# microsoft/M3P

Measured on AMD Instinct MI355X. Metric: pre-train samples/sec (whole node), 12L/768d seq=128+36, higher is better.
Workload: dtype bf16; 1 GPU; cfg2: 12L/768d/12h, 36 regions + 128 tokens, V=250002, 19 MLM targets/seq + ITM BCE, dropout 0.10, adam_inverse_sqrt + clip 5; per_gpu_batch=256, global_batch=256, seq_len=164, parallelism=dp1, prewarm_steps=36

## Files before the change

include/m3p_hip.h:

```cpp
#ifndef M3P_HIP_H
#define M3P_HIP_H

#include <stddef.h>
#include <stdint.h>

#ifdef __cplusplus
extern "C" {
#endif

#define M3P_API __attribute__((visibility("default")))

#define M3P_OK 0
#define M3P_EINVAL (-1)
#define M3P_ENOTIMPL (-2)
#define M3P_ENOMEM (-3)

M3P_API const char* m3p_version(void);


enum {
  M3P_EPI_NONE = 0,
  M3P_EPI_BIAS = 1,
  M3P_EPI_BIAS_GELU = 2,
  M3P_EPI_BIAS_DROP_RES = 3,
  M3P_EPI_RES = 4,
  M3P_EPI_DGELU = 5,
  M3P_EPI_MUL = 6,
  M3P_EPI_MULQ = 7,
  M3P_EPI_BIAS_GELUQ = 8,
  M3P_EPI_BIAS_LSE = 9
};

typedef struct M3PEpilogue {
  const float* bias;
  const void* aux;
  void* out2;
  float* colsum;
  int32_t ld_aux;
  int32_t ld_out2;
  int32_t scale_cols;
  float scale;
  float alpha;
  uint32_t seed;
  uint32_t thresh24;
  float inv_keep;
  const float* descale_a;
  const float* descale_b;
  void* out8;
  const float* scale8;
  float* amax8;
  int32_t ld_out8;
  int32_t out8_bf8;
} M3PEpilogue;

M3P_API int m3p_gemm_nt_bf16(const void* A, int lda, const void* W, int ldw, void* C, int ldc,
                             int M, int N, int K, int epilogue, const M3PEpilogue* ep, void* stream);

M3P_API int m3p_gemm_nt_fp8(const void* A8, int lda, int a_is_bf8, const void* W8, int ldw, void* C, int ldc,
                            int M, int N, int K, int epilogue, const M3PEpilogue* ep, void* stream);

M3P_API int m3p_quant_fp8(const void* src, int ld_src, void* dst, int ld_dst, int rows, int cols, const float* scale,
                          float* amax, int bf8, void* stream);

M3P_API int m3p_quant_fp8_batch(const long long* desc, int n_desc, int blocks_per_matrix, void* stream);

M3P_API int m3p_gemm_nt_streamk_f32(const void* A, int lda, const void* W, int ldw, float* C, int ldc,
                                    int M, int N, int K, float alpha, void* stream);
M3P_API int m3p_gemm_nn_streamk_f32(const void* A, int lda, const void* W, int ldw, int k_valid, float* C,
                                    int ldc, int M, int N, int K, float alpha, void* stream);
M3P_API int m3p_gemm_nn_w4_f32(const void* A, int lda, const void* W, int ldw, float* C, int ldc, int M, int N, int K, float alpha,
                               void* workspace, size_t workspace_bytes, void* stream);

M3P_API size_t m3p_gemm_wgrad_workspace_bytes(void);
M3P_API int m3p_gemm_wgrad_bf16(const void* dY, int lddy, const void* X, int ldx, float* dW, int lddw,
                                int M, int N, int K, float alpha, void* workspace, size_t workspace_bytes,
                                void* stream);
M3P_API int m3p_gemm_wgrad_store_bf16(const void* dY, int lddy, const void* X, int ldx, float* dW, int lddw, int M, int N, int K,
                                      float alpha, void* workspace, size_t workspace_bytes, void* stream);
M3P_API int m3p_gemm_wgrad_pair_bf16(const void* dYa, int lddya, const void* Xa, int ldxa, float* dWa, int lddwa, int Na, int Ka,
                                     const void* dYb, int lddyb, const void* Xb, int ldxb, float* dWb, int lddwb, int Nb, int Kb,
                                     int M, float alpha, void* workspace, size_t workspace_bytes, void* stream);


M3P_API int m3p_layernorm_fwd(const void* x, const float* gamma, const float* beta, const uint8_t* rowmask,
                              void* y, float* mean, float* rstd, int rows, int d, float eps, void* stream);

M3P_API int m3p_layernorm_bwd(const void* dy_a, const void* dy_b, const void* x, const float* gamma,
                              const float* mean, const float* rstd, const uint8_t* rowmask,
                              void* dx, void* dx_drop, float* dgamma, float* dbeta, float* dbias_drop,
                              int rows, int d, uint32_t seed, uint32_t thresh24, float inv_keep, void* stream);


M3P_API int m3p_attn_fwd(const void* qkv, const int32_t* keylen, void* ctx, float* lse, uint64_t* keepmask,
                         int B, int S, int H, int dh, uint32_t seed, uint32_t thresh24, float inv_keep,
                         void* stream);

M3P_API int m3p_attn_bwd(const void* qkv, const int32_t* keylen, const void* ctx, const void* dctx,
                         const float* lse, const uint64_t* keepmask, void* dqkv, float* dbias_qkv, int B, int S,
                         int H, int dh, float qscale, uint32_t seed, uint32_t thresh24, float inv_keep,
                         void* stream);

M3P_API int m3p_attn_query_fwd(const void* q, int ld_q, const void* kv, long long kv_bstride, int ld_kv,
                               const int32_t* klen, void* ctx, int B, int Tq, int H, int dh, int Lk, int causal,
                               int pos0, void* stream);

M3P_API int m3p_attn_rows_fwd(const void* q, int ld_q, const void* kv, long long kv_bstride, int ld_kv, const int32_t* klen,
                              void* ctx, float* lse, int B, int Tq, int H, int dh, int Lk, int causal, int pos0,
                              uint32_t seed, uint32_t thresh24, float inv_keep, void* stream);
M3P_API int m3p_attn_rows_bwd(const void* q, int ld_q, const void* kv, long long kv_bstride, int ld_kv, const int32_t* klen,
                              const void* dctx, const float* lse, void* dq, int ld_dq, float* dkv, int B, int Tq, int H,
                              int dh, int Lk, int causal, int pos0, float qscale, uint32_t seed, uint32_t thresh24,
                              float inv_keep, void* stream);


M3P_API int m3p_cast_f32_bf16(const float* src, void* dst, long long n, void* stream);

M3P_API int m3p_embed_assemble_fwd(const int64_t* tok, const void* emb_bf16, const float* pos,
                                   const void* img_proj, const float* loc, const float* w_loc,
                                   const float* b_loc, const float* g_img, const float* be_img,
                                   const float* g_emb, const float* be_emb, const int32_t* totlen,
                                   void* h, void* z, float* mean_emb, float* rstd_emb, void* e,
                                   float* mean_img, float* rstd_img, int B, int T, int R, int d,
                                   uint32_t seed_img, uint32_t seed_emb, uint32_t thresh24, float inv_keep,
                                   const void* img_rows, void* stream);

M3P_API int m3p_embed_image_rows_fwd(const void* img_proj, const float* loc, const float* w_loc, const float* b_loc,
                                     const float* g_img, const float* be_img, void* e, float* mean_img,
                                     float* rstd_img, void* img_rows, int B, int R, int d, uint32_t seed_img,
                                     uint32_t thresh24, float inv_keep, void* stream);

M3P_API int m3p_embed_assemble_bwd(const void* dh, const void* z, const float* mean_emb, const float* rstd_emb,
                                   const float* g_emb, const void* e, const float* mean_img,
                                   const float* rstd_img, const float* g_img, const int64_t* tok,
                                   const int32_t* totlen, const float* loc, void* dz_scratch, void* de,
                                   float* d_g_emb, float* d_be_emb, float* d_pos, float* d_emb,
                                   void* d_tok_rows, float* d_g_img, float* d_be_img, float* d_b_img, float* d_b_loc,
                                   float* d_w_loc, int B, int T, int R, int d, int pad_index,
                                   uint32_t seed_img, uint32_t seed_emb, uint32_t thresh24, float inv_keep,
                                   int phase, void* stream);


M3P_API int m3p_gather_rows(const void* src, const int32_t* idx, void* dst, int n, int d, void* stream);
M3P_API int m3p_scatter_add_rows(const void* src, const int32_t* idx, void* dst, int n, int d, void* stream);
M3P_API int m3p_scatter_add_token_rows(const void* rows, int ld_rows, const int64_t* ids, float* dst, int n, int d,
                                       int pad_index, void* stream);

M3P_API int m3p_itm_score_fwd(const void* pre, const float* w2, const float* b2, float* pooled, float* scores, int B,
                              int d, void* stream);
M3P_API int m3p_itm_score_bwd(const float* dscores, const float* pooled, const float* w2, void* dpre16, void* dpreT16,
                              int ldt, float* db1, float* dw2, float* db2, int B, int d, void* stream);

M3P_API int m3p_ce_fwd_bwd(void* logits, int ld, int n_rows, int V, const int64_t* target, float* row_loss,
                           float* loss_sum, float loss_scale, float grad_scale, void* stream);

M3P_API int m3p_ce_lse_from_blocks(const void* stats, int n_blocks, int n_rows, const void* logits, int ld, const int64_t* target,
                                   float* row_loss, float* row_lse, void* scratch, void* stream);
M3P_API int m3p_ce_bwd_colsum(void* logits, int ld, int n_rows, int V, const int64_t* target, const float* row_lse,
                              float grad_scale, float* colsum, void* workspace, size_t workspace_bytes, void* stream);
M3P_API size_t m3p_ce_colsum_workspace_bytes(int ld, int n_rows);
M3P_API int m3p_ce_fwd_bwd_colsum(void* logits, int ld, int n_rows, int V, const int64_t* target, float* row_loss,
                                  float* row_lse, float grad_scale, float* colsum, void* workspace,
                                  size_t workspace_bytes, void* stream);

M3P_API int m3p_colsum_bf16(const void* x, int ld, int n, int ncols, float* out, const float* scale_ptr,
                            void* stream);


M3P_API int m3p_sumsq_f32(const float* g, long long n, double* out, void* stream);

M3P_API int m3p_sumsq_ranges_f32(const float* base, const long long* starts, const long long* counts, int n_ranges, double* out,
                                 void* stream);

M3P_API int m3p_adam_step(float* p, float* g, float* m, float* v, void* w16, long long n, float lr, float beta1,
                          float beta2, float eps, float weight_decay, float step_size, const double* gnorm_sq,
                          float max_norm, float grad_scale, int zero_grad, void* stream);
M3P_API int m3p_adam_step_ranges(float* p, float* g, float* m, float* v, void* w16, const long long* starts,
                                 const long long* counts, const float* step_sizes, const int* zero_grad, int n_ranges,
                                 float lr, float beta1, float beta2, float eps, float weight_decay, const double* gnorm_sq,
                                 float max_norm, float grad_scale, void* stream);

M3P_API int m3p_gelu_fwd(const void* u, void* h, void* dh, long long n, void* stream);
M3P_API int m3p_gelu_fwd_gq(const void* u, void* h, void* gq, int M, int N, void* stream);
M3P_API int m3p_gelu_fwd_q8(const void* u, void* h, void* h8, long long n, const float* scale, float* amax, void* stream);

M3P_API int m3p_gelu_bwd(const void* dy, const void* u, void* du, long long n, void* stream);

M3P_API int m3p_mse_fwd_bwd(const void* pred, int ld_pred, const float* tgt, int ld_tgt, void* dpred, float* row_sq,
                            int rows, int cols, float grad_scale, void* stream);


M3P_API int m3p_dropout_rows(const void* x, int ldx, const void* res, int ldres, void* y, int ldy, int rows, int cols,
                             uint32_t rng_ld, uint32_t rng_col0, uint32_t seed, uint32_t thresh24, float inv_keep,
                             void* stream);

M3P_API int m3p_glu_fwd(const void* ab, int ld_ab, void* y, int rows, int d, void* stream);
// ... 51 lines not shown
```

m3p_amd/csrc/gemm.hip:

```cpp
#include <mutex>
#include <type_traits>
#include "common.hpp"
#include "../../include/m3p_hip.h"
#include <hip/amd_detail/amd_hip_unsafe_atomics.h>

static int g_variant = 1;
extern "C" void m3p_debug_set_variant(int v) { g_variant = (v == 2 || v == 6) ? v : 1; }

namespace {

constexpr int BK = 64;
constexpr int ROWB = BK * 2;

template <int EPI>
__device__ __forceinline__ void epilogue_store(const M3PEpilogue& ep, bf16* __restrict__ C, int ldc,
                                               int M, int N, int m, int n, f32x4 acc, f32x4& csum) {
  if (m >= M || n >= N) return;
  const bool full = (n + 3 < N);
  float v[4] = {acc[0], acc[1], acc[2], acc[3]};
  const float alpha = (ep.alpha == 0.f) ? 1.f : ep.alpha;
  if (EPI == M3P_EPI_NONE || EPI == M3P_EPI_BIAS || EPI == M3P_EPI_RES) {
#pragma unroll
    for (int r = 0; r < 4; ++r) v[r] *= alpha;
  }
  if (EPI == M3P_EPI_BIAS || EPI == M3P_EPI_BIAS_GELU || EPI == M3P_EPI_BIAS_DROP_RES) {
    if (ep.bias) {
#pragma unroll
      for (int r = 0; r < 4; ++r)
        if (n + r < N) v[r] += ep.bias[n + r];
    }
  }
  if (EPI == M3P_EPI_BIAS) {
#pragma unroll
    for (int r = 0; r < 4; ++r)
      if (n + r < ep.scale_cols) v[r] *= ep.scale;
  }
  if (EPI == M3P_EPI_BIAS_GELU) {
    bf16* U = reinterpret_cast<bf16*>(ep.out2) + (size_t)m * ep.ld_out2 + n;
    bf16 ur[4];
#pragma unroll
    for (int r = 0; r < 4; ++r) { ur[r] = (bf16)v[r]; v[r] = gelu_erf_f((float)ur[r]); }
    if (full) *reinterpret_cast<bf16x4*>(U) = bf16x4{ur[0], ur[1], ur[2], ur[3]};
    else
      for (int r = 0; r < 4; ++r) if (n + r < N) U[r] = ur[r];
  }
  if (EPI == M3P_EPI_BIAS_DROP_RES) {
    if (ep.thresh24) {
      const uint32_t base = (uint32_t)m * (uint32_t)N + (uint32_t)n;
      bool kp[4];
      m3p_keep_run<4>(base, ep.seed, ep.thresh24, kp);
#pragma unroll
      for (int r = 0; r < 4; ++r) v[r] = kp[r] ? v[r] * ep.inv_keep : 0.f;
    }
  }
  if (EPI == M3P_EPI_BIAS_DROP_RES || EPI == M3P_EPI_RES || EPI == M3P_EPI_DGELU || EPI == M3P_EPI_MUL) {
    const bf16* X = reinterpret_cast<const bf16*>(ep.aux) + (size_t)m * ep.ld_aux + n;
    float a[4] = {0.f, 0.f, 0.f, 0.f};
    if (full) { bf16x4 t = *reinterpret_cast<const bf16x4*>(X); a[0] = (float)t[0]; a[1] = (float)t[1]; a[2] = (float)t[2]; a[3] = (float)t[3]; }
    else
      for (int r = 0; r < 4; ++r) if (n + r < N) a[r] = (float)X[r];
    if (EPI == M3P_EPI_DGELU) {
#pragma unroll
      for (int r = 0; r < 4; ++r) v[r] *= gelu_erf_grad_f(a[r]);
    } else if (EPI == M3P_EPI_MUL) {
#pragma unroll
      for (int r = 0; r < 4; ++r) v[r] *= a[r];
    } else {
#pragma unroll
      for (int r = 0; r < 4; ++r) v[r] += a[r];
    }
  }
  bf16 o[4];
#pragma unroll
  for (int r = 0; r < 4; ++r) o[r] = (bf16)v[r];
  bf16* Cp = C + (size_t)m * ldc + n;
  if (full) *reinterpret_cast<bf16x4*>(Cp) = bf16x4{o[0], o[1], o[2], o[3]};
  else
    for (int r = 0; r < 4; ++r) if (n + r < N) Cp[r] = o[r];
  if (EPI == M3P_EPI_DGELU || EPI == M3P_EPI_MUL) {
#pragma unroll
    for (int r = 0; r < 4; ++r) csum[r] += (n + r < N) ? (float)o[r] : 0.f;
  }
}

template <int BM, int BN, int EPI>
__global__ __launch_bounds__(64 * (BM / 64) * (BN / 64))
void gemm_nt_kernel(const bf16* __restrict__ A, int lda, const bf16* __restrict__ W, int ldw,
                    bf16* __restrict__ C, int ldc, int M, int N, int K, M3PEpilogue ep,
                    int tiles_m, int tiles_n) {
  constexpr int WAVES_M = BM / 64, WAVES_N = BN / 64, NWAVES = WAVES_M * WAVES_N;
  constexpr int A_BYTES = BM * ROWB, B_BYTES = BN * ROWB, STAGE = A_BYTES + B_BYTES;
  extern __shared__ __attribute__((aligned(16))) char smem[];

  const int tid = threadIdx.x, lane = tid & 63;
  const int wid = __builtin_amdgcn_readfirstlane(tid >> 6);
  const int id = xcd_remap(blockIdx.x, tiles_m * tiles_n);
  const int tm = id / tiles_n, tn = id - tm * tiles_n;
  const int m0 = tm * BM, n0 = tn * BN;

  const int sr = lane >> 3, sc = (lane & 7) ^ sr;
  const bf16* a_src[BM / 8 / NWAVES];
// ... 150 lines not shown
template <class P>
__device__ __forceinline__ void st16(P* p, const u32x4& v) {
  *reinterpret_cast<u32x4*>(p) = v;
}
template <bool NT>
__device__ __forceinline__ void st16p(void* p, const u32x4& v) {
  if (NT) __builtin_nontemporal_store(v, reinterpret_cast<u32x4*>(p));
  else *reinterpret_cast<u32x4*>(p) = v;
}
template <int EPI>
__device__ __forceinline__ void load_aux_rows_issue(const M3PEpilogue& ep, int mrow0, int nw, int lane, u32x4 (&t)[4]) {
  constexpr bool kAux = (EPI == M3P_EPI_BIAS_DROP_RES || EPI == M3P_EPI_RES || EPI == M3P_EPI_DGELU || EPI == M3P_EPI_MUL);
  if (!kAux) return;
  const int srow = lane >> 3, sch = lane & 7;
  const bf16* X = reinterpret_cast<const bf16*>(ep.aux) + (size_t)(mrow0 + srow) * ep.ld_aux + nw + sch * 8;
#pragma unroll
  for (int it = 0; it < 4; ++it) {
    t[it] = *reinterpret_cast<const u32x4*>(X + (size_t)(it * 8) * ep.ld_aux);
  }
}
template <int EPI, bool SW = false, bool ALDS = false>
__device__ __forceinline__ void load_aux_rows_finish(int lane, char* r1, const u32x4 (&t)[4], bf16x4 (&auxv)[2][4]) {
  constexpr bool kAux = (EPI == M3P_EPI_BIAS_DROP_RES || EPI == M3P_EPI_RES || EPI == M3P_EPI_DGELU || EPI == M3P_EPI_MUL);
  if (!kAux) return;
  const int srow = lane >> 3, sch = lane & 7;
  const int fr = lane & 15, fg = lane >> 4;
  if (ALDS) {
    const uint32_t la = lds_addr(r1);
#pragma unroll
    for (int it = 0; it < 4; ++it) lds_w128(la + ep_off<SW>(it * 8 + srow, sch * 16), flip_halves(t[it], SW && (it & 1)));
#pragma unroll
    for (int ii = 0; ii < 2; ++ii)
#pragma unroll
      for (int j = 0; j < 4; ++j) lds_r64(la + ep_off8<SW>(ii * 16 + fr, (j * 16 + fg * 4) * 2), auxv[ii][j]);
    asm volatile("s_waitcnt lgkmcnt(0)" : "+v"(auxv[0][0]), "+v"(auxv[0][1]), "+v"(auxv[0][2]), "+v"(auxv[0][3]),
                                         "+v"(auxv[1][0]), "+v"(auxv[1][1]), "+v"(auxv[1][2]), "+v"(auxv[1][3]));
    return;
  }
#pragma unroll
  for (int it = 0; it < 4; ++it) *reinterpret_cast<u32x4*>(r1 + ep_off<SW>(it * 8 + srow, sch * 16)) = flip_halves(t[it], SW && (it & 1));
#pragma unroll
  for (int ii = 0; ii < 2; ++ii)
#pragma unroll
    for (int j = 0; j < 4; ++j)
      auxv[ii][j] = *reinterpret_cast<const bf16x4*>(r1 + ep_off8<SW>(ii * 16 + fr, (j * 16 + fg * 4) * 2));
}
template <int EPI, bool SW = false>
__device__ __forceinline__ void load_aux_rows(const M3PEpilogue& ep, int mrow0, int nw, int lane, char* r1, bf16x4 (&auxv)[2][4]) {
  u32x4 t[4];
  load_aux_rows_issue<EPI>(ep, mrow0, nw, lane, t);
  load_aux_rows_finish<EPI, SW>(lane, r1, t, auxv);
}

template <int EPI, bool SW = false, bool ALDS = false>
__device__ __forceinline__ void epilogue_half_write(const M3PEpilogue& ep, int N, int mrow0, int nw, char* r1, const f32x4 (&rows)[2][4],
                                                    const f32x4 (&biasv)[4], const bf16x4 (&auxv)[2][4], int lane, f32x4 (&csum)[4],
                                                    bf16x4 (&ukeep)[2][4], const float* gtab = nullptr) {
  const int fr = lane & 15, fg = lane >> 4;
  constexpr bool kAux = (EPI == M3P_EPI_BIAS_DROP_RES || EPI == M3P_EPI_RES || EPI == M3P_EPI_DGELU || EPI == M3P_EPI_MUL);
  const float alpha = (ep.alpha == 0.f) ? 1.f : ep.alpha;
#pragma unroll
  for (int j = 0; j < 4; ++j) {
    const int n = nw + j * 16 + fg * 4;
    f32x4 bias4 = biasv[j];
    f32x4 mulc = {alpha, alpha, alpha, alpha};
    if (EPI == M3P_EPI_BIAS) {
#pragma unroll
      for (int r = 0; r < 4; ++r)
        if (n + r < ep.scale_cols) { mulc[r] *= ep.scale; bias4[r] *= ep.scale; }
    }
#pragma unroll
    for (int ii = 0; ii < 2; ++ii) {
      const int rl = ii * 16 + fr;
      const int mrow = mrow0 + rl;
      const int lo = ep_off8<SW>(rl, (j * 16 + fg * 4) * 2);
      f32x4 v = rows[ii][j];
      if (EPI == M3P_EPI_NONE || EPI == M3P_EPI_BIAS || EPI == M3P_EPI_RES) v = v * mulc + bias4;
      else if (EPI != M3P_EPI_DGELU && EPI != M3P_EPI_MUL) v += bias4;
      if (EPI == M3P_EPI_BIAS_GELU) {
        ukeep[ii][j] = bf16x4{(bf16)v[0], (bf16)v[1], (bf16)v[2], (bf16)v[3]};
#pragma unroll
        for (int r = 0; r < 4; ++r) v[r] = gelu_erf_f((float)ukeep[ii][j][r]);
      }
      if (EPI == M3P_EPI_BIAS_DROP_RES && ep.thresh24) {
        const uint32_t base = (uint32_t)mrow * (uint32_t)N + (uint32_t)n;
        bool kp[4];
        m3p_keep_even<4>(base, ep.seed, ep.thresh24, kp);
#pragma unroll
        for (int r = 0; r < 4; ++r) v[r] = kp[r] ? v[r] * ep.inv_keep : 0.f;
      }
      if (kAux) {
        const bf16x4 t = auxv[ii][j];
        const f32x4 a = f32x4{(float)t[0], (float)t[1], (float)t[2], (float)t[3]};
        if (EPI == M3P_EPI_DGELU) {
          if (gtab) {
#pragma unroll
            for (int r = 0; r < 4; ++r) v[r] *= gelu_grad_lookup(gtab, t[r]);
          } else {
#pragma unroll
            for (int r = 0; r < 4; ++r) v[r] *= gelu_erf_grad_f(a[r]);
          }
        } else if (EPI == M3P_EPI_MUL) {
          v *= a;
        } else {
          v += a;
        }
      }
      const bf16x4 ob = bf16x4{(bf16)v[0], (bf16)v[1], (bf16)v[2], (bf16)v[3]};
      if (ALDS) lds_w64(lds_addr(r1) + lo, ob);
      else *reinterpret_cast<bf16x4*>(r1 + lo) = ob;
      if (EPI == M3P_EPI_DGELU || EPI == M3P_EPI_MUL) csum[j] += f32x4{(float)ob[0], (float)ob[1], (float)ob[2], (float)ob[3]};
    }
  }
}
template <bool SW>
__device__ __forceinline__ void epilogue_rows_read(const char* r1, int lane, u32x4 (&R)[4]) {
  const int srow = lane >> 3, sch = lane & 7;
  const uint32_t la = lds_addr(r1);
#pragma unroll
  for (int it = 0; it < 4; ++it) lds_r128(la + ep_off<SW>(it * 8 + srow, sch * 16), R[it]);
}
template <bool SW>
__device__ __forceinline__ void lgkm_wait_rows(u32x4 (&R)[4], bool younger8) {
  if (younger8) asm volatile("s_waitcnt lgkmcnt(8)" : "+v"(R[0]), "+v"(R[1]), "+v"(R[2]), "+v"(R[3]));
  else asm volatile("s_waitcnt lgkmcnt(0)" : "+v"(R[0]), "+v"(R[1]), "+v"(R[2]), "+v"(R[3]));
#pragma unroll
  for (int it = 0; it < 4; ++it) R[it] = flip_halves(R[it], SW && (it & 1));
}
__device__ __forceinline__ void epilogue_rows_store(bf16* __restrict__ C, int ldc, int mrow0, int nw, int lane, const u32x4 (&R)[4]) {
  const int srow = lane >> 3, sch = lane & 7;
  bf16* Cp = C + (size_t)mrow0 * ldc + nw + sch * 8;
#pragma unroll
  for (int it = 0; it < 4; ++it) st16(Cp + (size_t)(it * 8 + srow) * ldc, R[it]);
}
template <int EPI, bool SW = false>
__device__ __forceinline__ void epilogue_half(const M3PEpilogue& ep, bf16* __restrict__ C, int ldc, int N,
                                              int mrow0, int nw, char* r1, const f32x4 (&rows)[2][4],
                                              const f32x4 (&biasv)[4], const bf16x4 (&auxv)[2][4], int lane, f32x4 (&csum)[4],
// ... 1364 lines not shown
  } else {
    asm volatile("s_waitcnt vmcnt(0)" ::: "memory");
  }
  __builtin_amdgcn_s_barrier();
  asm volatile("" ::: "memory");
  bf16x8 af0[4], wf0[4], af1[4], wf1[4];
  s16x4 wh0[4][2], wh1[4][2];
  read_set(0, 0, af0, wf0, wh0);
  M3P_LGKM0();
  WgCursor cc = locate(g0l);
  int cur = 0;
  for (int step = 0; step < total; ++step) {
    const int nxt = (cur == 2) ? 0 : cur + 1;
    const int nx2 = (nxt == 2) ? 0 : nxt + 1;
    const bool more2 = (step + 2 < total);
    if (more2) stage_next(nx2);
    read_set(1, cur * STAGE, af1, wf1, wh1);
    __builtin_amdgcn_sched_barrier(0);
    mfma_batch(af0, wf0, wh0);
    M3P_LGKM0();
    if (more2) asm volatile("s_waitcnt vmcnt(6)" ::: "memory");
    else asm volatile("s_waitcnt vmcnt(0)" ::: "memory");
    __builtin_amdgcn_s_barrier();
    asm volatile("" ::: "memory");
    __builtin_amdgcn_sched_barrier(0);
    read_set(0, nxt * STAGE, af0, wf0, wh0);
    __builtin_amdgcn_sched_barrier(0);
    mfma_batch(af1, wf1, wh1);
    M3P_LGKM0();
    if ((cc.mt + 1 == cc.len) || (step + 1 == total)) {
      const int tm = cc.t / tiles_n, tn = cc.t - tm * tiles_n;
#pragma unroll
      for (int i = 0; i < 4; ++i) {
        const int m = tm * BM + wm * 64 + i * 16 + fr;
#pragma unroll
        for (int j = 0; j < 4; ++j) {
          const int n = tn * BN + wn * 64 + j * 16 + fg * 4;
#pragma unroll
          for (int r = 0; r < 4; ++r) {
            if (m < M && n + r < N) unsafeAtomicAdd(Cf + (size_t)m * ldc + n + r, alpha * acc[i][j][r]);
            acc[i][j][r] = 0.f;
          }
        }
      }
    }
    advance(cc);
    cur = nxt;
  }
#undef M3P_DSR
#undef M3P_TRH
#undef M3P_LGKM0
}

template <int EPI>
__global__ __launch_bounds__(256)
void gemm_nt_w4_kernel(const bf16* __restrict__ A, int lda, const bf16* __restrict__ W, int ldw,
                       bf16* __restrict__ C, int ldc, int M, int N, int K, M3PEpilogue ep,
                       int tiles_m, int tiles_n, int m_fast) {
  constexpr int BM = 256, BN = 256, KT = 64;
  constexpr int A_BYTES = BM * KT * 2, STAGE = (BM + BN) * KT * 2;
  extern __shared__ __attribute__((aligned(16))) char smem[];

  const int tid = threadIdx.x, lane = tid & 63;
  const int wid = __builtin_amdgcn_readfirstlane(tid >> 6);
  const int ntiles = tiles_m * tiles_n;
  const int n_strips = (tiles_n >= 12) ? (tiles_n + 3) / 4 : 1;
  const int strip_w = (tiles_n + n_strips - 1) / n_strips;
  auto split_tile = [&](int t, int& tm, int& tn) {
    if (m_fast) { tn = t / tiles_m; tm = t - tn * tiles_m; return; }
    const int strip = t / (tiles_m * strip_w);
    const int rem = t - strip * tiles_m * strip_w;
    const int bn = min(strip_w, tiles_n - strip * strip_w);
    tm = rem / bn;
    tn = strip * strip_w + (rem - tm * bn);
  };
  const int nwg = gridDim.x;
  const int per_xcd = nwg >> 3;
  const int slot = (blockIdx.x & 7) * per_xcd + (blockIdx.x >> 3);
  auto tile_of = [&](int q) { return q * nwg + slot; };
  const int my_tiles = (ntiles > slot) ? (ntiles - slot + nwg - 1) / nwg : 0;
  if (my_tiles == 0) return;
  const int nk = K / KT;
  const int total = my_tiles * nk;

  const int l_row = lane >> 3;
  const int l_col = ((lane & 7) ^ l_row) * 8;
  const uint32_t a_lane = (uint32_t)(l_row * lda + l_col) * 2u, w_lane = (uint32_t)(l_row * ldw + l_col) * 2u;
  __amdgpu_buffer_rsrc_t a_rsrc, w_rsrc;
  int l_q = 0, l_kt = 0;
  auto set_load_tile = [&](int q) {
    int tm, tn;
    split_tile(tile_of(q), tm, tn);
    const bf16* a_tile = A + (size_t)(tm * BM + wid * 64) * lda;
    const bf16* w_tile = W + (size_t)(tn * BN + wid * 64) * ldw;
    a_rsrc = __builtin_amdgcn_make_buffer_rsrc(const_cast<bf16*>(uniform_ptr(a_tile)), 0, 0xffffffff, 0x00020000);
    w_rsrc = __builtin_amdgcn_make_buffer_rsrc(const_cast<bf16*>(uniform_ptr(w_tile)), 0, 0xffffffff, 0x00020000);
  };
#define W4_LDB(IMM) __builtin_amdgcn_raw_ptr_buffer_load_lds(piece < 8 ? a_rsrc : w_rsrc, LDS_PTR(sl), 16, piece < 8 ? a_lane : w_lane, soff, IMM, 0)
  auto issue_load = [&](int s, int piece) {
    const int pc = piece & 7;
    char* sl = smem + s * STAGE + (piece < 8 ? 0 : A_BYTES) + wid * 8192 + (pc >> 2) * 4096;
    const uint32_t k_off = (uint32_t)l_kt * (KT * 2);
    const uint32_t soff = __builtin_amdgcn_readfirstlane(k_off + (uint32_t)pc * (uint32_t)((piece < 8 ? lda : ldw) * 16) - (uint32_t)(pc & 3) * 1024u);
    switch (pc & 3) {
      case 0: W4_LDB(0); break;
      case 1: W4_LDB(1024); break;
      case 2: W4_LDB(2048); break;
      default: W4_LDB(3072); break;
    }
  };
  auto load_done = [&]() {
// ... 204 lines not shown
        load_bias4<EPI>(ep, btn * BN + wn * 128 + 64, lane, bias_hi);
      }
      ktile(std::true_type{}, stage_c);
    } else {
      ktile(std::false_type{}, stage_c);
    }
    if (++c_kt == nk) {
      c_kt = 0;
      asm volatile("s_nop 15\n\ts_nop 15" ::: "memory");
      int tm, tn;
      split_tile(tile_of(c_q), tm, tn);
      ++c_q;
      const int m0 = tm * BM, n0 = tn * BN;
      const int mw = m0 + wm * 128, nw = n0 + wn * 128;
      const bool fast = io_aligned && (m0 + BM <= M) && (n0 + BN <= N);
      f32x4 csum[4];
#pragma unroll
      for (int j = 0; j < 4; ++j) csum[j] = f32x4{0.f, 0.f, 0.f, 0.f};
#define W4_RD(II, JJ, I, J)                                                         \
  asm volatile("v_accvgpr_read_b32 %0, a[((" #I ")*8+(" #J "))*4+0]\n\t"            \
               "v_accvgpr_read_b32 %1, a[((" #I ")*8+(" #J "))*4+1]\n\t"            \
               "v_accvgpr_read_b32 %2, a[((" #I ")*8+(" #J "))*4+2]\n\t"            \
               "v_accvgpr_read_b32 %3, a[((" #I ")*8+(" #J "))*4+3]"                \
               : "=v"(t0), "=v"(t1), "=v"(t2), "=v"(t3));                           \
  rows[II][JJ] = f32x4{t0, t1, t2, t3}
#define W4_SLICE(RG, CH)                                                                      \
  W4_RD(0, 0, 2 * RG, 4 * CH); W4_RD(0, 1, 2 * RG, 4 * CH + 1); W4_RD(0, 2, 2 * RG, 4 * CH + 2); W4_RD(0, 3, 2 * RG, 4 * CH + 3); \
  W4_RD(1, 0, 2 * RG + 1, 4 * CH); W4_RD(1, 1, 2 * RG + 1, 4 * CH + 1); W4_RD(1, 2, 2 * RG + 1, 4 * CH + 2); W4_RD(1, 3, 2 * RG + 1, 4 * CH + 3)
      constexpr bool kPipe = (EPI == M3P_EPI_NONE || EPI == M3P_EPI_BIAS || EPI == M3P_EPI_RES || EPI == M3P_EPI_BIAS_DROP_RES);
      if (kPipe && fast) {
        char* rb = smem + 2 * STAGE + wid * EP_HALF;
        u32x4 tq[4];
        load_aux_rows_issue<EPI>(ep, mw, nw, lane, tq);
#pragma nounroll
        for (int p = 0; p < 8; ++p) {
          const int ch = p >> 2, rg = p & 3;
          f32x4 rows[2][4];
          float t0, t1, t2, t3;
          switch (p) {
            case 0: W4_SLICE(0, 0); break;
            case 1: W4_SLICE(1, 0); break;
            case 2: W4_SLICE(2, 0); break;
            case 3: W4_SLICE(3, 0); break;
            case 4: W4_SLICE(0, 1); break;
            case 5: W4_SLICE(1, 1); break;
            case 6: W4_SLICE(2, 1); break;
            default: W4_SLICE(3, 1); break;
          }
          char* rc = rb;
          bf16x4 aux_cur[2][4];
          load_aux_rows_finish<EPI, true, true>(lane, rc, tq, aux_cur);
          if (p + 1 < 8) load_aux_rows_issue<EPI>(ep, mw + 32 * ((p + 1) & 3), nw + 64 * ((p + 1) >> 2), lane, tq);
          bf16x4 ukeep[2][4];
          epilogue_half_write<EPI, true, true>(ep, N, mw + 32 * rg, nw + 64 * ch, rc, rows, ch ? bias_hi : bias_lo, aux_cur, lane, csum, ukeep);
          u32x4 R[4];
          epilogue_rows_read<true>(rc, lane, R);
          lgkm_wait_rows<true>(R, false);
          epilogue_rows_store(C, ldc, mw + 32 * rg, nw + 64 * ch, lane, R);
        }
      } else
#pragma nounroll
      for (int p = 0; p < 8; ++p) {
        const int ch = p >> 2, rg = p & 3;
        bf16x4 aux_cur[2][4];
        if (fast) {
          if (EPI == M3P_EPI_DGELU || EPI == M3P_EPI_MUL) load_aux<EPI>(ep, mw + 32 * rg, nw + 64 * ch, lane, aux_cur);
          else load_aux_rows<EPI>(ep, mw + 32 * rg, nw + 64 * ch, lane, r1, aux_cur);
        }
        f32x4 rows[2][4];
        float t0, t1, t2, t3;
        switch (p) {
          case 0: W4_SLICE(0, 0); break;
          case 1: W4_SLICE(1, 0); break;
          case 2: W4_SLICE(2, 0); break;
          case 3: W4_SLICE(3, 0); break;
          case 4: W4_SLICE(0, 1); break;
          case 5: W4_SLICE(1, 1); break;
          case 6: W4_SLICE(2, 1); break;
          default: W4_SLICE(3, 1); break;
        }
        const int mrow0 = mw + 32 * rg, ncol0 = nw + 64 * ch;
        if (fast) {
          epilogue_half<EPI>(ep, C, ldc, N, mrow0, ncol0, r1, rows, ch ? bias_hi : bias_lo, aux_cur, lane, csum);
        } else {
#pragma unroll
          for (int ii = 0; ii < 2; ++ii)
#pragma unroll
            for (int jj = 0; jj < 4; ++jj)
              epilogue_store<EPI>(ep, C, ldc, M, N, mrow0 + ii * 16 + fr, ncol0 + jj * 16 + fg * 4, rows[ii][jj], csum[jj]);
        }
        if ((EPI == M3P_EPI_DGELU || EPI == M3P_EPI_MUL) && rg == 3) {
          if (ep.colsum) {
#pragma unroll
            for (int j = 0; j < 4; ++j)
#pragma unroll
              for (int r = 0; r < 4; ++r) {
                float sfl = csum[j][r];
                sfl += __shfl_xor(sfl, 1, 64); sfl += __shfl_xor(sfl, 2, 64);
                sfl += __shfl_xor(sfl, 4, 64); sfl += __shfl_xor(sfl, 8, 64);
                const int n = ncol0 + j * 16 + fg * 4 + r;
                if (fr == 0 && n < N) unsafeAtomicAdd(ep.colsum + n, sfl);
              }
          }
#pragma unroll
          for (int j = 0; j < 4; ++j) csum[j] = f32x4{0.f, 0.f, 0.f, 0.f};
        }
      }
// ... 141 lines not shown
int launch_nt(const bf16* A, int lda, const bf16* W, int ldw, bf16* C, int ldc, int M, int N, int K,
              const M3PEpilogue& ep, hipStream_t st) {
  int want_queue = 0;
  const int plan = nt_plan(EPI, M, N, K, &want_queue);
  if (plan == M3P_KERN_NT_SKINNY) {
    if constexpr (EPI != M3P_EPI_DGELU && EPI != M3P_EPI_MUL) {
      if (M <= 16) return launch_nt_skinny<EPI, 1>(A, lda, W, ldw, C, ldc, M, N, K, ep, st);
      if (M <= 32) return launch_nt_skinny<EPI, 2>(A, lda, W, ldw, C, ldc, M, N, K, ep, st);
      if (M <= 64) return launch_nt_skinny<EPI, 4>(A, lda, W, ldw, C, ldc, M, N, K, ep, st);
      return launch_nt_skinny<EPI, 8>(A, lda, W, ldw, C, ldc, M, N, K, ep, st);
    }
  }
  if (plan == M3P_KERN_NT_W8) {
    const int tiles_m = M / 256, tiles_n = N / 256;
    const size_t lds = 2 * 512 * ROWB + (EPI == M3P_EPI_DGELU ? GELU_TAB_N * sizeof(float) : 0) +
                       ((EPI == M3P_EPI_DGELU || EPI == M3P_EPI_MUL) ? 8 * 2048 : 8 * 4096);
    auto kern = gemm_nt_w8_kernel<EPI>;
    static bool attr_set8 = false;
    if (!attr_set8) {
      hipError_t e = hipFuncSetAttribute((const void*)kern, hipFuncAttributeMaxDynamicSharedMemorySize, (int)lds);
      if (e != hipSuccess) return (int)e;
      attr_set8 = true;
    }
    int grid = num_cus();
    const int ntiles = tiles_m * tiles_n;
    if (ntiles < grid) grid = (ntiles + 7) / 8 * 8;
    constexpr bool kQueueOk = !(EPI == M3P_EPI_DGELU || EPI == M3P_EPI_MUL);
    int* ctr = nullptr;
    if (kQueueOk && want_queue) {
      hipError_t e;
      ctr = tq_acquire(st, &e);
      if (e != hipSuccess) return (int)e;
    }
    if constexpr (kQueueOk) if (ctr) {
      auto kern_d = gemm_nt_w8_kernel<EPI, true>;
      static bool attr_set8d = false;
      if (!attr_set8d) {
        hipError_t e = hipFuncSetAttribute((const void*)kern_d, hipFuncAttributeMaxDynamicSharedMemorySize, (int)lds);
        if (e != hipSuccess) return (int)e;
        attr_set8d = true;
      }
      hipLaunchKernelGGL(kern_d, dim3(grid), dim3(512), lds, st, A, lda, W, ldw, C, ldc, M, N, K, ep, tiles_m, tiles_n, ctr);
      M3P_CHECK_LAUNCH();
      return M3P_OK;
    }
    hipLaunchKernelGGL(kern, dim3(grid), dim3(512), lds, st, A, lda, W, ldw, C, ldc, M, N, K, ep, tiles_m, tiles_n, ctr);
    M3P_CHECK_LAUNCH();
    return M3P_OK;
  }
  if (plan == M3P_KERN_NT_W4) {
    constexpr int BM = 256, BN = 256;
    const int tiles_m = (M + BM - 1) / BM, tiles_n = (N + BN - 1) / BN;
    const size_t lds = 2 * (BM + BN) * 128 + 4 * EP_HALF;
    auto kern = gemm_nt_w4_kernel<EPI>;
    static bool attr_set = false;
    if (!attr_set) {
      hipError_t e = hipFuncSetAttribute((const void*)kern, hipFuncAttributeMaxDynamicSharedMemorySize, (int)lds);
      if (e != hipSuccess) return (int)e;
      attr_set = true;
    }
    int grid = num_cus();
    const int ntiles = tiles_m * tiles_n;
    if (ntiles < grid) grid = (ntiles + 7) / 8 * 8;
    const long long wbytes = 2LL * N * K, abytes = 2LL * M * K;
    const int m_fast = (wbytes > (64LL << 20) && abytes < wbytes) ? 1 : 0;
    hipLaunchKernelGGL(kern, dim3(grid), dim3(256), lds, st, A, lda, W, ldw, C, ldc, M, N, K, ep, tiles_m, tiles_n, m_fast);
    M3P_CHECK_LAUNCH();
    return M3P_OK;
  }
  if (plan == M3P_KERN_NT_RING) {
    constexpr int BM = 256, BN = 128;
    const int tiles_m = (M + BM - 1) / BM, tiles_n = (N + BN - 1) / BN;
    const size_t lds = 3 * (BM + BN) * ROWB + (EPI == M3P_EPI_DGELU ? GELU_TAB_N * sizeof(float) : 0);
    auto kern = gemm_nt_ring_kernel<EPI>;
    static bool attr_set = false;
    if (!attr_set) {
      hipError_t e = hipFuncSetAttribute((const void*)kern, hipFuncAttributeMaxDynamicSharedMemorySize, (int)lds);
      if (e != hipSuccess) return (int)e;
      attr_set = true;
    }
    int grid = num_cus();
    const int ntiles = tiles_m * tiles_n;
    if (ntiles < grid) grid = (ntiles + 7) / 8 * 8;
    hipLaunchKernelGGL(kern, dim3(grid), dim3(512), lds, st, A, lda, W, ldw, C, ldc, M, N, K, ep, tiles_m, tiles_n);
    M3P_CHECK_LAUNCH();
    return M3P_OK;
  }
  constexpr int BM = 128, BN = 128;
  const int tiles_m = (M + BM - 1) / BM, tiles_n = (N + BN - 1) / BN;
  const size_t lds = 2 * (BM + BN) * ROWB;
  auto kern = gemm_nt_kernel<BM, BN, EPI>;
  static bool attr_set = false;
  if (!attr_set) {
    hipError_t e = hipFuncSetAttribute((const void*)kern, hipFuncAttributeMaxDynamicSharedMemorySize, (int)lds);
    if (e != hipSuccess) return (int)e;
    attr_set = true;
  }
  hipLaunchKernelGGL(kern, dim3(tiles_m * tiles_n), dim3(256), lds, st, A, lda, W, ldw, C, ldc, M, N, K, ep,
                     tiles_m, tiles_n);
  M3P_CHECK_LAUNCH();
  return M3P_OK;
}

template <int EPI>
static int launch_nt_gq(const bf16* A, int lda, const bf16* W, int ldw, bf16* C, int ldc, int M, int N, int K,
                        const M3PEpilogue& ep, hipStream_t st) {
  if (M < 1024 || (M % 256) || (N % 256) || N < 512 || (K % 64) || (lda % 8) || (ldw % 8) || (ldc % 8) || ((uintptr_t)C & 15))
    return M3P_EINVAL;
// ... 1081 lines not shown
```

m3p_amd/csrc/heads.hip:

```cpp
#include "common.hpp"
#include <hip/amd_detail/amd_hip_unsafe_atomics.h>

namespace {

__global__ __launch_bounds__(256) void gather_rows_kernel(const bf16* __restrict__ src, const int32_t* __restrict__ idx,
                                                          bf16* __restrict__ dst, int n, int d) {
  const int nchunk = d >> 2;
  const size_t total = (size_t)n * nchunk;
  for (size_t i = (size_t)blockIdx.x * blockDim.x + threadIdx.x; i < total; i += (size_t)gridDim.x * blockDim.x) {
    const int r = (int)(i / nchunk), c = (int)(i - (size_t)r * nchunk);
    *reinterpret_cast<bf16x4*>(dst + (size_t)r * d + 4 * c) =
        *reinterpret_cast<const bf16x4*>(src + (size_t)idx[r] * d + 4 * c);
  }
}
__global__ __launch_bounds__(256) void scatter_add_rows_kernel(const bf16* __restrict__ src, const int32_t* __restrict__ idx,
                                                               bf16* __restrict__ dst, int n, int d) {
  const int nchunk = d >> 2;
  const size_t total = (size_t)n * nchunk;
  for (size_t i = (size_t)blockIdx.x * blockDim.x + threadIdx.x; i < total; i += (size_t)gridDim.x * blockDim.x) {
    const int r = (int)(i / nchunk), c = (int)(i - (size_t)r * nchunk);
    bf16* p = dst + (size_t)idx[r] * d + 4 * c;
    Vec4<bf16>::store(p, Vec4<bf16>::load(p) + Vec4<bf16>::load(src + (size_t)r * d + 4 * c));
  }
}

__global__ __launch_bounds__(256) void scatter_add_token_rows_kernel(const bf16* __restrict__ rows, int ld_rows, const int64_t* __restrict__ ids,
                                                                     float* __restrict__ dst, int n, int d, int pad_index) {
  const int lane = threadIdx.x & 63;
  const int wave = (int)((blockIdx.x * blockDim.x + threadIdx.x) >> 6), nwave = (int)((gridDim.x * blockDim.x) >> 6);
  for (int r = wave; r < n; r += nwave) {
    const int64_t id = ids[r];
    if (id == pad_index) continue;
    const bf16* src = rows + (size_t)r * ld_rows;
    float* out = dst + (size_t)id * d;
    for (int e = lane; e < d; e += 64) {
      const float v = (float)src[e];
      if (v != 0.f) unsafeAtomicAdd(out + e, v);
    }
  }
}

__global__ __launch_bounds__(1024) void ce_fwd_bwd_kernel(bf16* __restrict__ logits, int ld, int V,
                                                          const int64_t* __restrict__ target, float* __restrict__ row_loss,
                                                          float* __restrict__ loss_sum, float loss_scale, float gscale) {
  __shared__ float s_m[16], s_s[16];
  constexpr float kLog2e = 1.4426950408889634f;
  const int row = blockIdx.x, tid = threadIdx.x, lane = tid & 63, wib = tid >> 6;
  bf16* lr = logits + (size_t)row * ld;
  const int nchunk = ld >> 3;
  float m = -INFINITY, s = 0.f;
  for (int c = tid; c < nchunk; c += 1024) {
    const bf16x8 v = *reinterpret_cast<const bf16x8*>(lr + 8 * c);
    float x[8];
    float gm = -INFINITY;
#pragma unroll
    for (int j = 0; j < 8; ++j) {
      x[j] = (8 * c + j < V) ? (float)v[j] : -INFINITY;
      gm = fmaxf(gm, x[j]);
    }
    if (gm > m) {
      s *= __builtin_amdgcn_exp2f((m - gm) * kLog2e);
      m = gm;
    }
    const float mb = m * kLog2e;
#pragma unroll
// ... 219 lines not shown

int m3p_ce_lse_from_blocks(const void* stats, int n_blocks, int n_rows, const void* logits, int ld, const int64_t* target,
                           float* row_loss, float* row_lse, void* scratch, void* stream) {
  if (n_blocks <= 0 || n_rows <= 0 || (n_rows % 64) != 0 || !stats || !logits || !target || !row_loss || !row_lse || !scratch ||
      ((uintptr_t)stats & 7) || ((uintptr_t)scratch & 7))
    return M3P_EINVAL;
  hipStream_t st = (hipStream_t)stream;
  hipLaunchKernelGGL(ce_lse_partial_kernel, dim3(n_rows / 64, CE_LSE_SPLIT), dim3(256), 0, st, (const float2*)stats, n_blocks, n_rows,
                     (float2*)scratch);
  hipLaunchKernelGGL(ce_lse_final_kernel, dim3((n_rows + 255) / 256), dim3(256), 0, st, (const float2*)scratch, n_rows,
                     (const bf16*)logits, ld, target, row_loss, row_lse);
  M3P_CHECK_LAUNCH();
  return M3P_OK;
}

int m3p_ce_bwd_colsum(void* logits, int ld, int n_rows, int V, const int64_t* target, const float* row_lse,
                      float grad_scale, float* colsum, void* workspace, size_t workspace_bytes, void* stream) {
  if (n_rows <= 0 || V <= 0 || ld < V || (ld % 8) != 0 || ((uintptr_t)logits & 15) || ((uintptr_t)colsum & 15) ||
      ((uintptr_t)workspace & 15) || !row_lse)
    return M3P_EINVAL;
  if (workspace_bytes < m3p_ce_colsum_workspace_bytes(ld, n_rows)) return M3P_EINVAL;
  hipStream_t st = (hipStream_t)stream;
  const int groups = (n_rows + CE_RB - 1) / CE_RB;
  hipLaunchKernelGGL(ce_grad_tile_kernel, dim3((ld + CE_CB - 1) / CE_CB, groups), dim3(256), 0, st, (bf16*)logits, ld, n_rows, V,
                     target, (const float*)row_lse, grad_scale, (float*)workspace);
  if (hipMemsetAsync(colsum, 0, (size_t)ld * sizeof(float), st) != hipSuccess) return M3P_EINVAL;
  hipLaunchKernelGGL(ce_colsum_reduce_kernel, dim3((ld / 4 + 255) / 256, groups >= 16 ? 8 : 1), dim3(256), 0, st,
                     (const float*)workspace, ld, groups, colsum);
  M3P_CHECK_LAUNCH();
  return M3P_OK;
}

int m3p_colsum_bf16(const void* x, int ld, int n, int ncols, float* out, const float* scale_ptr, void* stream) {
  if (n <= 0 || ncols <= 0 || (ld % 4) != 0 || ld < ((ncols + 3) / 4) * 4) return M3P_EINVAL;
  const int c4 = (ncols + 3) / 4;
  int ysplit = 1;
  while (ysplit < 64 && ((c4 + 255) / 256) * ysplit < 1024 && n / (ysplit * 2) >= 16) ysplit *= 2;
  hipLaunchKernelGGL(colsum_kernel, dim3((c4 + 255) / 256, ysplit), dim3(256), 0, (hipStream_t)stream, (const bf16*)x, ld,
                     n, ncols, out, scale_ptr);
  M3P_CHECK_LAUNCH();
  return M3P_OK;
}

int m3p_gather_rows(const void* src, const int32_t* idx, void* dst, int n, int d, void* stream) {
  if (n <= 0) return M3P_OK;
  if ((d % 4) != 0) return M3P_EINVAL;
  const size_t total = (size_t)n * (d / 4);
  const int blocks = (int)((total + 255) / 256 < 2048 ? (total + 255) / 256 : 2048);
  hipLaunchKernelGGL(gather_rows_kernel, dim3(blocks), dim3(256), 0, (hipStream_t)stream, (const bf16*)src, idx, (bf16*)dst, n, d);
  M3P_CHECK_LAUNCH();
  return M3P_OK;
}

int m3p_scatter_add_rows(const void* src, const int32_t* idx, void* dst, int n, int d, void* stream) {
  if (n <= 0) return M3P_OK;
  if ((d % 4) != 0) return M3P_EINVAL;
  const size_t total = (size_t)n * (d / 4);
  const int blocks = (int)((total + 255) / 256 < 2048 ? (total + 255) / 256 : 2048);
  hipLaunchKernelGGL(scatter_add_rows_kernel, dim3(blocks), dim3(256), 0, (hipStream_t)stream, (const bf16*)src, idx, (bf16*)dst, n, d);
  M3P_CHECK_LAUNCH();
  return M3P_OK;
}

int m3p_scatter_add_token_rows(const void* rows, int ld_rows, const int64_t* ids, float* dst, int n, int d, int pad_index, void* stream) {
  if (n <= 0) return M3P_OK;
  if (d <= 0 || ld_rows < d) return M3P_EINVAL;
  const int blocks = (n + 3) / 4 < 4096 ? (n + 3) / 4 : 4096;
  hipLaunchKernelGGL(scatter_add_token_rows_kernel, dim3(blocks), dim3(256), 0, (hipStream_t)stream, (const bf16*)rows, ld_rows, ids,
                     dst, n, d, pad_index);
  M3P_CHECK_LAUNCH();
  return M3P_OK;
}

int m3p_ce_fwd_bwd(void* logits, int ld, int n_rows, int V, const int64_t* target, float* row_loss, float* loss_sum,
                   float loss_scale, float grad_scale, void* stream) {
  if (n_rows <= 0 || V <= 0 || ld < V || (ld % 8) != 0 || ((uintptr_t)logits & 15)) return M3P_EINVAL;
  hipLaunchKernelGGL(ce_fwd_bwd_kernel, dim3(n_rows), dim3(1024), 0, (hipStream_t)stream, (bf16*)logits, ld, V, target,
                     row_loss, loss_sum, loss_scale, grad_scale);
  M3P_CHECK_LAUNCH();
  return M3P_OK;
}

}
```

m3p_amd/csrc/layernorm.hip:

```cpp
#include "common.hpp"
#include "../../include/m3p_hip.h"
#include <hip/amd_detail/amd_hip_unsafe_atomics.h>

namespace {

constexpr int LN_BWD_BLOCKS = 512;

template <int NI>
__global__ __launch_bounds__(256)
void ln_fwd_kernel(const bf16* __restrict__ x, const float* __restrict__ gamma, const float* __restrict__ beta,
                   const uint8_t* __restrict__ rowmask, bf16* __restrict__ y, float* __restrict__ mean,
                   float* __restrict__ rstd, int rows, int d, float eps) {
  const int lane = threadIdx.x & 63;
  const int wave = (blockIdx.x * blockDim.x + threadIdx.x) >> 6;
  const int nwaves = (gridDim.x * blockDim.x) >> 6;
  const int nchunk = d >> 2;
  const float inv_d = 1.0f / (float)d;

  f32x4 g[NI], b[NI];
#pragma unroll
  for (int i = 0; i < NI; ++i) {
    const int c = lane + 64 * i;
    if (c < nchunk) { g[i] = Vec4<float>::load(gamma + 4 * c); b[i] = Vec4<float>::load(beta + 4 * c); }
  }
  for (int r = wave; r < rows; r += nwaves) {
    const bf16* xr = x + (size_t)r * d;
    f32x4 v[NI];
    float s = 0.f;
#pragma unroll
    for (int i = 0; i < NI; ++i) {
      const int c = lane + 64 * i;
      v[i] = f32x4{0.f, 0.f, 0.f, 0.f};
      if (c < nchunk) v[i] = Vec4<bf16>::load(xr + 4 * c);
      s += (v[i][0] + v[i][1]) + (v[i][2] + v[i][3]);
    }
    const float mu = wave_sum(s) * inv_d;
    float q = 0.f;
#pragma unroll
    for (int i = 0; i < NI; ++i) {
      const int c = lane + 64 * i;
      if (c < nchunk) {
        const f32x4 t = v[i] - mu;
        q += (t[0] * t[0] + t[1] * t[1]) + (t[2] * t[2] + t[3] * t[3]);
      }
    }
    const float rs = 1.0f / sqrtf(wave_sum(q) * inv_d + eps);
    const float mk = rowmask ? (rowmask[r] ? 1.f : 0.f) : 1.f;
    bf16* yr = y + (size_t)r * d;
#pragma unroll
    for (int i = 0; i < NI; ++i) {
      const int c = lane + 64 * i;
      if (c < nchunk) {
        f32x4 o = ((v[i] - mu) * rs * g[i] + b[i]) * mk;
        Vec4<bf16>::store(yr + 4 * c, o);
      }
    }
    if (lane == 0) { mean[r] = mu; rstd[r] = rs; }
  }
}

template <int NI>
__global__ __launch_bounds__(256)
void ln_bwd_kernel(const bf16* __restrict__ dy_a, const bf16* __restrict__ dy_b, const bf16* __restrict__ x,
                   const float* __restrict__ gamma, const float* __restrict__ mean, const float* __restrict__ rstd,
                   const uint8_t* __restrict__ rowmask, bf16* __restrict__ dx, bf16* __restrict__ dx_drop,
                   float* __restrict__ dgamma, float* __restrict__ dbeta, float* __restrict__ dbias_drop,
                   int rows, int d, uint32_t seed, uint32_t thresh24, float inv_keep) {
  __shared__ float red[4][NI * 256];
  const int lane = threadIdx.x & 63, wib = threadIdx.x >> 6;
  const int wave = (blockIdx.x * blockDim.x + threadIdx.x) >> 6;
  const int nwaves = (gridDim.x * blockDim.x) >> 6;
  const int nchunk = d >> 2;
  const float inv_d = 1.0f / (float)d;

  f32x4 g[NI], acc_g[NI], acc_b[NI], acc_d[NI];
#pragma unroll
  for (int i = 0; i < NI; ++i) {
    const int c = lane + 64 * i;
    g[i] = f32x4{0.f, 0.f, 0.f, 0.f};
    if (c < nchunk) g[i] = Vec4<float>::load(gamma + 4 * c);
    acc_g[i] = acc_b[i] = acc_d[i] = f32x4{0.f, 0.f, 0.f, 0.f};
  }
  for (int r = wave; r < rows; r += nwaves) {
    const size_t ro = (size_t)r * d;
    const float mu = mean[r], rs = rstd[r];
    const float mk = rowmask ? (rowmask[r] ? 1.f : 0.f) : 1.f;
    f32x4 dyv[NI], xh[NI];
    float s1 = 0.f, s2 = 0.f;
#pragma unroll
    for (int i = 0; i < NI; ++i) {
      const int c = lane + 64 * i;
      dyv[i] = xh[i] = f32x4{0.f, 0.f, 0.f, 0.f};
      if (c < nchunk) {
        dyv[i] = Vec4<bf16>::load(dy_a + ro + 4 * c);
        if (dy_b) dyv[i] += Vec4<bf16>::load(dy_b + ro + 4 * c);
        dyv[i] *= mk;
        xh[i] = (Vec4<bf16>::load(x + ro + 4 * c) - mu) * rs;
        const f32x4 gd = dyv[i] * g[i];
        s1 += (gd[0] + gd[1]) + (gd[2] + gd[3]);
        const f32x4 gx = gd * xh[i];
        s2 += (gx[0] + gx[1]) + (gx[2] + gx[3]);
        acc_g[i] += dyv[i] * xh[i];
        acc_b[i] += dyv[i];
      }
    }
    const float c1 = wave_sum(s1) * inv_d, c2 = wave_sum(s2) * inv_d;
#pragma unroll
    for (int i = 0; i < NI; ++i) {
      const int c = lane + 64 * i;
      if (c < nchunk) {
        const f32x4 o = (dyv[i] * g[i] - c1 - xh[i] * c2) * rs;
        Vec4<bf16>::store(dx + ro + 4 * c, o);
        if (dx_drop || dbias_drop) {
          bf16x4 ob = bf16x4{(bf16)o[0], (bf16)o[1], (bf16)o[2], (bf16)o[3]};
          f32x4 od;
          const uint32_t base = (uint32_t)r * (uint32_t)d + 4u * (uint32_t)c;
          bool kp[4] = {true, true, true, true};
          if (thresh24) m3p_keep_even<4>(base, seed, thresh24, kp);
#pragma unroll
          for (int e = 0; e < 4; ++e) od[e] = kp[e] ? (float)ob[e] * (thresh24 ? inv_keep : 1.f) : 0.f;
          bf16x4 odb = bf16x4{(bf16)od[0], (bf16)od[1], (bf16)od[2], (bf16)od[3]};
          if (dx_drop) *reinterpret_cast<bf16x4*>(dx_drop + ro + 4 * c) = odb;
          acc_d[i] += f32x4{(float)odb[0], (float)odb[1], (float)odb[2], (float)odb[3]};
        }
      }
    }
  }
  float* const outs[3] = {dgamma, dbeta, dbias_drop};
#pragma unroll
  for (int q = 0; q < 3; ++q) {
    if (outs[q] == nullptr) continue;
#pragma unroll
    for (int i = 0; i < NI; ++i) {
      const int col = 4 * (lane + 64 * i);
      const f32x4 a = (q == 0) ? acc_g[i] : (q == 1) ? acc_b[i] : acc_d[i];
#pragma unroll
      for (int e = 0; e < 4; ++e) red[wib][col + e] = a[e];
    }
    __syncthreads();
    for (int c = threadIdx.x; c < d; c += blockDim.x)
      unsafeAtomicAdd(outs[q] + c, (red[0][c] + red[1][c]) + (red[2][c] + red[3][c]));
    __syncthreads();
  }
}

template <int NC>
__global__ __launch_bounds__(256)
void ln_bwd_hw_kernel(const bf16* __restrict__ dy_a, const bf16* __restrict__ dy_b, const bf16* __restrict__ x,
                      const float* __restrict__ gamma, const float* __restrict__ mean, const float* __restrict__ rstd,
                      const uint8_t* __restrict__ rowmask, bf16* __restrict__ dx, bf16* __restrict__ dx_drop,
                      float* __restrict__ dgamma, float* __restrict__ dbeta, float* __restrict__ dbias_drop,
                      int rows, uint32_t seed, uint32_t thresh24, float inv_keep) {
  constexpr int D = 256 * NC;
  __shared__ float red[8][D];
  const int sub = threadIdx.x & 31, hw = threadIdx.x >> 5;
  const int ghw = blockIdx.x * 8 + hw, nhw = gridDim.x * 8;
  const float inv_d = 1.0f / (float)D;
  float g[NC][8], acc_g[NC][8], acc_b[NC][8], acc_d[NC][8];
#pragma unroll
  for (int i = 0; i < NC; ++i) {
    const int c = (sub + 32 * i) * 8;
    const f32x4 g0 = Vec4<float>::load(gamma + c), g1 = Vec4<float>::load(gamma + c + 4);
#pragma unroll
    for (int e = 0; e < 4; ++e) { g[i][e] = g0[e]; g[i][4 + e] = g1[e]; }
#pragma unroll
    for (int e = 0; e < 8; ++e) acc_g[i][e] = acc_b[i][e] = acc_d[i][e] = 0.f;
  }
  auto hsum = [](float v) {
#pragma unroll
    for (int o = 16; o > 0; o >>= 1) v += __shfl_xor(v, o, 64);
    return v;
  };
  for (int r = ghw; r < rows; r += nhw) {
    const size_t ro = (size_t)r * D;
    const float mu = mean[r], rs = rstd[r];
    const float mk = rowmask ? (rowmask[r] ? 1.f : 0.f) : 1.f;
    float dyv[NC][8], xh[NC][8];
    float s1 = 0.f, s2 = 0.f;
#pragma unroll
    for (int i = 0; i < NC; ++i) {
      const int c = (sub + 32 * i) * 8;
      bf16x8 a = *reinterpret_cast<const bf16x8*>(dy_a + ro + c);
      const bf16x8 xv = *reinterpret_cast<const bf16x8*>(x + ro + c);
      bf16x8 b2;
      if (dy_b) b2 = *reinterpret_cast<const bf16x8*>(dy_b + ro + c);
#pragma unroll
      for (int e = 0; e < 8; ++e) {
        float dv = (float)a[e];
        if (dy_b) dv += (float)b2[e];
        dv *= mk;
        const float xe = ((float)xv[e] - mu) * rs;
        dyv[i][e] = dv; xh[i][e] = xe;
        const float gd = dv * g[i][e];
        s1 += gd; s2 += gd * xe;
        acc_g[i][e] += dv * xe;
        acc_b[i][e] += dv;
      }
    }
    const float c1 = hsum(s1) * inv_d, c2 = hsum(s2) * inv_d;
#pragma unroll
    for (int i = 0; i < NC; ++i) {
      const int c = (sub + 32 * i) * 8;
      bf16x8 ob, odb;
#pragma unroll
      for (int e = 0; e < 8; ++e) ob[e] = (bf16)((dyv[i][e] * g[i][e] - c1 - xh[i][e] * c2) * rs);
      *reinterpret_cast<bf16x8*>(dx + ro + c) = ob;
      if (dx_drop || dbias_drop) {
        const uint32_t base = (uint32_t)r * (uint32_t)D + (uint32_t)c;
        bool kp[8] = {true, true, true, true, true, true, true, true};
        if (thresh24) m3p_keep_even<8>(base, seed, thresh24, kp);
#pragma unroll
        for (int e = 0; e < 8; ++e) {
          odb[e] = (bf16)(kp[e] ? (float)ob[e] * (thresh24 ? inv_keep : 1.f) : 0.f);
          acc_d[i][e] += (float)odb[e];
        }
        if (dx_drop) *reinterpret_cast<bf16x8*>(dx_drop + ro + c) = odb;
      }
    }
  }
  float* const outs[3] = {dgamma, dbeta, dbias_drop};
#pragma unroll
  for (int q = 0; q < 3; ++q) {
    if (outs[q] == nullptr) continue;
#pragma unroll
    for (int i = 0; i < NC; ++i) {
      const int c = (sub + 32 * i) * 8;
#pragma unroll
      for (int e = 0; e < 8; ++e) red[hw][c + e] = (q == 0) ? acc_g[i][e] : (q == 1) ? acc_b[i][e] : acc_d[i][e];
    }
    __syncthreads();
    for (int c = threadIdx.x; c < D; c += 256) {
      float t = 0.f;
#pragma unroll
      for (int w = 0; w < 8; ++w) t += red[w][c];
      unsafeAtomicAdd(outs[q] + c, t);
    }
    __syncthreads();
  }
}

inline int ln_ni(int d) { return (d + 255) / 256; }

}

extern "C" {

int m3p_layernorm_fwd(const void* x, const float* gamma, const float* beta, const uint8_t* rowmask, void* y,
                      float* mean, float* rstd, int rows, int d, float eps, void* stream) {
  if (rows <= 0 || d <= 0 || (d % 4) != 0 || d > 2048) return M3P_EINVAL;
  if (((uintptr_t)x & 7) || ((uintptr_t)y & 7) || ((uintptr_t)gamma & 15) || ((uintptr_t)beta & 15)) return M3P_EINVAL;
  const int blocks = min((rows + 3) / 4, 4096);
  hipStream_t st = (hipStream_t)stream;
#define M3P_LN_FWD(NI)                                                                                  \
  hipLaunchKernelGGL(ln_fwd_kernel<NI>, dim3(blocks), dim3(256), 0, st, (const bf16*)x, gamma, beta,    \
                     rowmask, (bf16*)y, mean, rstd, rows, d, eps)
  switch (ln_ni(d)) {
    case 1: M3P_LN_FWD(1); break;
    case 2: M3P_LN_FWD(2); break;
    case 3: M3P_LN_FWD(3); break;
    case 4: M3P_LN_FWD(4); break;
    default: M3P_LN_FWD(8); break;
  }
#undef M3P_LN_FWD
  M3P_CHECK_LAUNCH();
  return M3P_OK;
}

int m3p_layernorm_bwd(const void* dy_a, const void* dy_b, const void* x, const float* gamma, const float* mean,
                      const float* rstd, const uint8_t* rowmask, void* dx, void* dx_drop, float* dgamma,
                      float* dbeta, float* dbias_drop, int rows, int d, uint32_t seed, uint32_t thresh24,
                      float inv_keep, void* stream) {
  if (rows <= 0 || d <= 0 || (d % 4) != 0 || d > 2048) return M3P_EINVAL;
  if (!dy_a || !x || !dx || !dgamma || !dbeta) return M3P_EINVAL;
  if (((uintptr_t)x & 7) || ((uintptr_t)dy_a & 7) || ((uintptr_t)dx & 7) || ((uintptr_t)gamma & 15)) return M3P_EINVAL;
  hipStream_t st = (hipStream_t)stream;
  if ((d == 768 || d == 1024) && !(((uintptr_t)x | (uintptr_t)dy_a | (uintptr_t)dx | (uintptr_t)dy_b | (uintptr_t)dx_drop) & 15)) {
    const int blocks_hw = min((rows + 7) / 8, LN_BWD_BLOCKS);
    if (d == 768)
      hipLaunchKernelGGL(ln_bwd_hw_kernel<3>, dim3(blocks_hw), dim3(256), 0, st, (const bf16*)dy_a, (const bf16*)dy_b,
                         (const bf16*)x, gamma, mean, rstd, rowmask, (bf16*)dx, (bf16*)dx_drop, dgamma, dbeta, dbias_drop,
                         rows, seed, thresh24, inv_keep);
    else
      hipLaunchKernelGGL(ln_bwd_hw_kernel<4>, dim3(blocks_hw), dim3(256), 0, st, (const bf16*)dy_a, (const bf16*)dy_b,
                         (const bf16*)x, gamma, mean, rstd, rowmask, (bf16*)dx, (bf16*)dx_drop, dgamma, dbeta, dbias_drop,
                         rows, seed, thresh24, inv_keep);
    M3P_CHECK_LAUNCH();
    return M3P_OK;
  }
  const int blocks = min((rows + 3) / 4, 512);
#define M3P_LN_BWD(NI)                                                                                     \
  hipLaunchKernelGGL(ln_bwd_kernel<NI>, dim3(blocks), dim3(256), 0, st, (const bf16*)dy_a,                 \
                     (const bf16*)dy_b, (const bf16*)x, gamma, mean, rstd, rowmask, (bf16*)dx,              \
                     (bf16*)dx_drop, dgamma, dbeta, dbias_drop, rows, d, seed, thresh24, inv_keep)
  switch (ln_ni(d)) {
    case 1: M3P_LN_BWD(1); break;
    case 2: M3P_LN_BWD(2); break;
    case 3: M3P_LN_BWD(3); break;
    case 4: M3P_LN_BWD(4); break;
    default: M3P_LN_BWD(8); break;
  }
#undef M3P_LN_BWD
  M3P_CHECK_LAUNCH();
  return M3P_OK;
}

}
```

m3p_amd/functional.py:

```python
import math
import os
from collections import OrderedDict

import torch

from . import lib as L
from . import fp8 as fp8mod
from . import ops
from . import rng

BF16 = torch.bfloat16
ALIGN = 64
BUCKET_ALIGN = 64 * 8


def _round_up(n, a):
    return (n + a - 1) // a * a


_VOCAB_FULL_TILES = os.environ.get('M3P_VOCAB_FULL_TILES', '1') != '0'
_GELU_GRAD_IN_FWD = os.environ.get('M3P_GELU_GRAD_IN_FWD', '0') != '0'
_GELU_BYTE_GRAD = int(os.environ.get('M3P_GELU_BYTE_GRAD', '2'))
_CE_FUSED_LSE = os.environ.get('M3P_CE_FUSED_LSE', '1') != '0'
_VOCAB_DGRAD_W4 = os.environ.get('M3P_VOCAB_DGRAD_W4', '1') != '0'
# ... 344 lines not shown
        del dy, dab, dcat, dctx, dxn_cat, dqkv, dxn, dln, dx1
    ar.touch(*[n for n in ar.names if n.startswith('refine_embeddings.')])
    return dx


class GradSink:

    def __init__(self):
        self.buf = None

    def rows(self, like):
        if self.buf is None:
            self.buf = torch.zeros_like(like)
        assert self.buf.shape == like.shape
        return self.buf

    def take(self):
        buf, self.buf = self.buf, None
        return buf


def _sink_of(tensor, base):
    root = tensor._base if tensor._is_view() else tensor
    sink = getattr(root, '_m3p_sink', None) if root is not None else None
    if sink is None or base is None or not torch.is_grad_enabled():
        return None
    if root.dim() != 2 or not root.is_contiguous() or root.storage_offset() != 0 or tuple(root.shape) != tuple(base.shape):
        return None
    return sink


def first_rows_sink(model, tensor):
    d = model.dim
    if tensor.dim() != 3 or tensor.dtype != BF16 or not tensor._is_view():
        return None, None, None
    st, soff = tensor.stride(), tensor.storage_offset()
    if st[2] != 1 or st[0] % d or soff % d:
        return None, None, None
    with torch.no_grad():
        base = torch.as_strided(tensor, (tensor.untyped_storage().nbytes() // 2 // d, d), (d, 1), 0)
    sink = _sink_of(tensor, base)
    if sink is None:
        return None, None, None
    cache = model.__dict__.setdefault('_first_rows_cache', {})
    key = (tensor.shape[0], st[0], soff, tensor.device)
    rows = cache.get(key)
    if rows is None:
        rows = ((soff + torch.arange(tensor.shape[0], device=tensor.device, dtype=torch.int64) * st[0]) // d).to(torch.int32)
        cache.clear()
        cache[key] = rows
    return sink, base, rows


N_ENC_ARGS = 16


class EncoderFn(torch.autograd.Function):

    @staticmethod
    def forward(ctx, anchor, model, x, lengths, x_img, lengths_img, image_loc, p_drop, p_attn, seed_step, p_refine=None,
                track=False, text_embed=None, langs=None, h0=None, positions=None):
        ar = model.arena()
        ready = model.ddp_hook.params_ready if model.ddp_hook is not None else (lambda key: None)
        ar.refresh(wait_params=False)
        ready('vocab')
        ready('embed')
        dev = ar.device
        d, H, nL = model.dim, model.n_heads, model.n_layers
        dh = d // H
        seed = lambda kind, i=0: rng.stream_seed(model.base_seed, seed_step, _site(kind, i))
        if h0 is not None:
            assert x is None and x_img is None and text_embed is None and langs is None and positions is None
            B = lengths.shape[0]
            S = h0.shape[0] // B
            T, R, M = S, 0, B * S
            totlen, rowmask = ops.seq_masks(lengths.to(device=dev, dtype=torch.int64).contiguous(), None, B, S)
            h = h0.detach().to(BF16).contiguous()
            ximg16 = loc = emb_saved = img_rows = img_saved = ref_saved = keylen_img = tok = None
        else:
            h = None
            T, B = x.shape
            R = 0 if x_img is None else x_img.shape[0]
            S = R + T
            M = B * S
            x = x.to(dev).contiguous()
        if h is None:
            table, tok = ar.w('embeddings.weight'), x
            if text_embed is not None:
                assert tuple(text_embed.shape) == (B, T, d), (tuple(text_embed.shape), (B, T, d))
                table = text_embed.detach().to(device=dev, dtype=BF16).contiguous().view(B * T, d)
                tok = (torch.arange(B, device=dev, dtype=torch.int64) * T)[None, :] + \
                    torch.arange(T, device=dev, dtype=torch.int64)[:, None]
                tok = tok.contiguous()
            if langs is not None or positions is not None:
                assert text_embed is None and R == 0
                rows = table[x.t()].float()
                if langs is not None:
                    langs = langs.to(dev).contiguous()
                    rows = rows + ar.p('cross_lang_embeddings.weight')[langs.t()]
                if positions is not None:
                    positions = positions.to(dev).contiguous()
                    assert positions.size() == (T, B)
                    ptab = ar.p('position_embeddings.weight')
                    rows = rows + ptab[positions.t()] - ptab[:T][None, :, :]
                table = rows.to(BF16).reshape(B * T, d).contiguous()
                tok = ((torch.arange(B, device=dev, dtype=torch.int64) * T)[None, :] +
                       torch.arange(T, device=dev, dtype=torch.int64)[:, None]).contiguous()
            totlen, rowmask = ops.seq_masks(lengths.to(device=dev, dtype=torch.int64).contiguous(),
                                            None if R == 0 else lengths_img.to(device=dev, dtype=torch.int64).contiguous(), B, S)

            ximg16 = img_proj = loc = None
            if R > 0:
                xi = x_img.detach().to(dev)
                if xi.dtype == torch.float32 and xi.stride(2) == 1 and xi.stride(0) % 4 == 0 and xi.stride(1) % 4 == 0:
                    ximg16 = ops.cast_rows_bf16(xi)
                else:
                    ximg16 = ops.cast_bf16(xi.contiguous().view(R * B, 2048))
                loc = image_loc.contiguous().float()
                img_proj = ops.gemm_nt(ximg16, ar.w('image_embeddings.image_embeddings.weight'), L.EPI_BIAS,
                                       bias=ar.p('image_embeddings.image_embeddings.bias'))
            img_rows = img_saved = ref_saved = keylen_img = None
            if p_refine is not None and R > 0:
                rows, img_saved = ops.embed_image_rows_fwd(
                    img_proj, loc, ar.p('image_embeddings.image_location_embeddings.weight'),
                    ar.p('image_embeddings.image_location_embeddings.bias'), ar.p('image_embeddings.LayerNorm.weight'),
                    ar.p('image_embeddings.LayerNorm.bias'), B, R, d, seed_img=seed('img'), p_drop=p_drop)
                keylen_img = lengths_img.to(device=dev, dtype=torch.int32).contiguous()
                img_rows, ref_saved = refiner_fwd(model, rows, keylen_img, B, R, seed_step, p_refine)
            h, emb_saved = ops.embed_assemble_fwd(
                tok, table, ar.p('position_embeddings.weight'), img_proj, loc,
                ar.p('image_embeddings.image_location_embeddings.weight'),
                ar.p('image_embeddings.image_location_embeddings.bias'),
                ar.p('image_embeddings.LayerNorm.weight'), ar.p('image_embeddings.LayerNorm.bias'),
                ar.p('layer_norm_emb.weight'), ar.p('layer_norm_emb.bias'), totlen, B, T, R, d,
                seed_img=seed('img'), seed_emb=seed('emb'), p_drop=p_drop, img_rows=img_rows, img_saved=img_saved)

        saved_layers = []
        qscale = 1.0 / math.sqrt(dh)
        st8 = model.fp8_state() if model.fp8 else None
        if st8 is not None:
            assert M % 256 == 0, 'the fp8 GEMM takes whole 256-row tiles (B * S %% 256 == 0): M = %d' % M
            if model.training:
                st8.roll()
            ready(None)
            st8.quant_weights(ar)

        def lin(xin, i, xsite, wsite, w16, epi, pre8=None, **kw):
            if st8 is None or wsite not in fp8mod.FWD_SITES:
                return ops.gemm_nt(xin, w16, epi, **kw)
            x8, dxs = pre8 if pre8 is not None else st8.quant(xin, i, xsite)
            w8, _, dws = st8.weights[(i, wsite)]
            return ops.gemm_nt_fp8(x8, w8, epi, descale_a=dxs, descale_b=dws, **kw)

        for i in range(nL):
            a, f = 'attentions.%d.' % i, 'ffns.%d.' % i
            ready(('layer', i))
            qkv = lin(h, i, 'x', 'wqkv', ar.qkv_w16(i), L.EPI_BIAS, bias=ar.qkv_bias(i), scale_cols=d, scale=qscale)
            ctxt, lse, kmask = ops.attn_fwd(qkv, totlen, B, S, H, dh, seed=seed('attn_p', i), p_drop=p_attn,
                                            want_mask=True)
            lse = (lse, kmask)
            pre1 = lin(ctxt, i, 'ctx', 'wout', ar.w(a + 'out_lin.weight'), L.EPI_BIAS_DROP_RES, bias=ar.p(a + 'out_lin.bias'),
                       aux=h, seed=seed('attn_out', i), p_drop=p_drop)
            x1, mean1, rstd1 = ops.layernorm_fwd(pre1, ar.p('layer_norm1.%d.weight' % i), ar.p('layer_norm1.%d.bias' % i))
            hact8 = None
            u_holds_grad = False
            if (st8 is None or 'w1' not in fp8mod.FWD_SITES) and not _GELU_GRAD_IN_FWD and _GELU_BYTE_GRAD == 2 and track \
                    and ops.gq_eligible(M, 4 * d):
                u = torch.empty((M * 4 * d,), dtype=torch.uint8, device=dev)
                o8 = {}
                if st8 is not None and 'w2' in fp8mod.FWD_SITES:
                    kh = st8.index(i, 'hact')
                    if st8.seen[kh]:
                        o8 = dict(out8=torch.empty((M, 4 * d), dtype=torch.uint8, device=dev), scale8=st8.scale[kh:kh + 1],
                                  amax8=st8.amax[kh:kh + 1])
                hact = ops.gemm_nt(x1, ar.w(f + 'lin1.weight'), L.EPI_BIAS_GELUQ, bias=ar.p(f + 'lin1.bias'), out2=u, **o8)
                if o8:
                    hact8 = (o8['out8'], st8.descale[kh:kh + 1])
                elif st8 is not None and 'w2' in fp8mod.FWD_SITES:
                    st8._first_use(hact, kh)
                u_holds_grad = 'q'
            elif M >= 1024 or st8 is not None:
                u = lin(x1, i, 'x1', 'w1', ar.w(f + 'lin1.weight'), L.EPI_BIAS, bias=ar.p(f + 'lin1.bias'))
                if st8 is not None and 'w2' in fp8mod.FWD_SITES and 'w2' not in fp8mod.BWD_SITES and not _GELU_GRAD_IN_FWD:
                    hact, hact8 = st8.gelu_quant(u, i)
                elif st8 is None and not _GELU_GRAD_IN_FWD and _GELU_BYTE_GRAD and track and ops.gq_eligible(M, 4 * d):
                    hact, u = ops.gelu_fwd_gq(u)
                    u_holds_grad = 'q'
                else:
                    u_holds_grad = _GELU_GRAD_IN_FWD or (st8 is not None and 'w2' in fp8mod.BWD_SITES)
                    hact = ops.gelu_fwd(u, grad_inplace=u_holds_grad)
            else:
                u = torch.empty((M, 4 * d), dtype=BF16, device=dev)
                hact = ops.gemm_nt(x1, ar.w(f + 'lin1.weight'), L.EPI_BIAS_GELU, bias=ar.p(f + 'lin1.bias'), out2=u)
            pre2 = lin(hact, i, 'hact', 'w2', ar.w(f + 'lin2.weight'), L.EPI_BIAS_DROP_RES, bias=ar.p(f + 'lin2.bias'),
                       aux=x1, seed=seed('ffn', i), p_drop=p_drop, pre8=hact8)
            h_next, mean2, rstd2 = ops.layernorm_fwd(pre2, ar.p('layer_norm2.%d.weight' % i),
                                                     ar.p('layer_norm2.%d.bias' % i), rowmask)
            if track:
                saved_layers.append((h, qkv, ctxt, lse, pre1, mean1, rstd1, x1, u, hact, pre2, mean2, rstd2))
            h = h_next

        ctx.model = model
        ctx.dims = (B, T, R, S, d, H, dh, nL)
        ctx.drop = (p_drop, p_attn, seed_step)
        ctx.u_holds_grad = nL > 0 and u_holds_grad
        ctx.saved = (tok if text_embed is not None else x, totlen, rowmask, ximg16, loc, emb_saved, saved_layers)
        ctx.refine = (ref_saved, keylen_img, p_refine)
        ctx.input_grads = (R > 0 and x_img.requires_grad and track, text_embed is not None)
        ctx.langs = langs
        ctx.positions = positions
        ctx.h0_mode = None if h0 is None else h0.dtype
        hook = model.ddp_hook
        ctx.track = bool(track) and hook is not None
        ctx.tok_rows_max = hook.encoder_forward(0 if h0 is not None else T * B) if ctx.track else None
        ctx.set_materialize_grads(False)
        ctx.sink = GradSink()
        model._pending_sink = ctx.sink
        return h

    @staticmethod
    def backward(ctx, dout):
        model = ctx.model
        ar = model.arena()
        B, T, R, S, d, H, dh, nL = ctx.dims
        M = B * S
        p_drop, p_attn, seed_step = ctx.drop
        x, totlen, rowmask, ximg16, loc, emb_saved, saved_layers = ctx.saved
        ctx.saved = None
        seed = lambda kind, i=0: rng.stream_seed(model.base_seed, seed_step, _site(kind, i))
        ref_saved, keylen_img, p_refine = ctx.refine
        ctx.refine = None
        hook = model.ddp_hook if ctx.track else None
        if model.ddp_hook is not None:
            model.ddp_hook.params_ready(None)
        sunk = ctx.sink.take()
        if dout is None and sunk is None:
            if hook is not None:
                hook.encoder_backward_end()
            return (None,) * N_ENC_ARGS
        if dout is None:
            dh_ = sunk
        else:
            dh_ = dout.contiguous()
            if dh_.dtype != BF16:
                dh_ = dh_.to(BF16)
            if sunk is not None:
                dh_ = dh_ + sunk.view_as(dh_)
        last = hook.encoder_backward_begin() if hook is not None else True
        st8 = model.fp8_state() if model.fp8 else None

        def dgrad(g, i, gsite, wsite, wt16, epi, pre8=None, **kw):
            if st8 is None or wsite not in fp8mod.BWD_SITES:
                return ops.gemm_nt(g, wt16, epi, **kw)
            g8, dgs = pre8 if pre8 is not None else st8.quant(g, i, gsite)
            _, wt8, dws = st8.weights[(i, wsite)]
            return ops.gemm_nt_fp8(g8, wt8, epi, a_is_bf8=True, descale_a=dgs, descale_b=dws, **kw)

        for i in reversed(range(nL)):
            a, f = 'attentions.%d.' % i, 'ffns.%d.' % i
            (h_in, qkv, ctxt, lse, pre1, mean1, rstd1, x1, u, hact, pre2, mean2, rstd2) = saved_layers[i]
            saved_layers[i] = None
            dpre2, dY2 = ops.layernorm_bwd(dh_, None, pre2, ar.p('layer_norm2.%d.weight' % i), mean2, rstd2, rowmask,
                                           ar.g('layer_norm2.%d.weight' % i), ar.g('layer_norm2.%d.bias' % i),
                                           dbias_drop=ar.g(f + 'lin2.bias'), want_drop=p_drop > 0,
                                           seed=seed('ffn', i), p_drop=p_drop)
            if dY2 is None:
                dY2 = dpre2
            ops.gemm_wgrad(dY2, hact, ar.g(f + 'lin2.weight'))
            du8 = None
            if ctx.u_holds_grad == 'q':
                o8 = {}
                if st8 is not None and 'w1' in fp8mod.BWD_SITES:
                    kd = st8.index(i, 'du')
                    if st8.seen[kd]:
                        o8 = dict(out8=torch.empty((M, 4 * d), dtype=torch.uint8, device=dY2.device), scale8=st8.scale[kd:kd + 1],
                                  amax8=st8.amax[kd:kd + 1], out8_bf8=True)
                dU = ops.gemm_nt(dY2, ar.wt[('lin2', i)], L.EPI_MULQ, aux=u, colsum=ar.g(f + 'lin1.bias'), **o8)
                if o8:
                    du8 = (o8['out8'], st8.descale[kd:kd + 1])
                elif st8 is not None and 'w1' in fp8mod.BWD_SITES:
                    st8._first_use(dU, kd)
            else:
                dU = dgrad(dY2, i, 'dy2', 'w2', ar.wt[('lin2', i)], L.EPI_MUL if ctx.u_holds_grad else L.EPI_DGELU, aux=u,
                           colsum=ar.g(f + 'lin1.bias'))
            del hact, u, pre2
            ops.gemm_wgrad(dU, x1, ar.g(f + 'lin1.weight'))
            dx1 = dgrad(dU, i, 'du', 'w1', ar.wt[('lin1', i)], L.EPI_RES, aux=dpre2, pre8=du8)
            del dU, dpre2, dY2
            dpre1, dAO = ops.layernorm_bwd(dx1, None, pre1, ar.p('layer_norm1.%d.weight' % i), mean1, rstd1, None,
                                           ar.g('layer_norm1.%d.weight' % i), ar.g('layer_norm1.%d.bias' % i),
                                           dbias_drop=ar.g(a + 'out_lin.bias'), want_drop=p_drop > 0,
                                           seed=seed('attn_out', i), p_drop=p_drop)
            if dAO is None:
                dAO = dpre1
            dctx = dgrad(dAO, i, 'dao', 'wout', ar.wt[('out', i)], L.EPI_NONE)
            dqkv = ops.attn_bwd(qkv, totlen, ctxt, dctx, lse[0], B, S, H, dh, dbias_qkv=ar.qkv_bias(i, grad=True),
                                seed=seed('attn_p', i), p_drop=p_attn, keepmask=lse[1])
            ops.gemm_wgrad_pair(dqkv, h_in, ar.qkv_wgrad(i), dAO, ctxt, ar.g(a + 'out_lin.weight'))
            dh_ = dgrad(dqkv, i, 'dqkv', 'wqkv', ar.wt[('qkv', i)], L.EPI_RES, aux=dpre1)
            del dqkv, dctx, dAO, dpre1, dx1
            ar.touch_layer(i)
            if hook is not None:
                hook.layer_done(i, last)
        if ctx.h0_mode is not None:
            if hook is not None:
                hook.embed_done(last, ids=None, rows=None, n_max=ctx.tok_rows_max)
            return (None,) * 14 + (dh_.to(ctx.h0_mode), None)
        want_dximg, has_text_embed = ctx.input_grads
        langs, positions = ctx.langs, ctx.positions
        tok_rows = None
        if has_text_embed or langs is not None or positions is not None or (hook is not None and hook.active):
            tok_rows = torch.empty((T * B, d), dtype=BF16, device=dh_.device)
        grads = dict(
            d_g_emb=ar.g('layer_norm_emb.weight'), d_be_emb=ar.g('layer_norm_emb.bias'),
            d_pos=ar.g('position_embeddings.weight'), d_emb=ar.g('embeddings.weight'),
            d_g_img=ar.g('image_embeddings.LayerNorm.weight'), d_be_img=ar.g('image_embeddings.LayerNorm.bias'),
            d_b_img=ar.g('image_embeddings.image_embeddings.bias'),
            d_b_loc=ar.g('image_embeddings.image_location_embeddings.bias'),
            d_w_loc=ar.g('image_embeddings.image_location_embeddings.weight'))
        de = ops.embed_assemble_bwd(dh_, emb_saved, ar.p('layer_norm_emb.weight'),
                                    ar.p('image_embeddings.LayerNorm.weight'), x, totlen, loc, grads, B, T, R, d,
                                    -1 if has_text_embed else model.pad_index, seed_img=seed('img'), seed_emb=seed('emb'), p_drop=p_drop,
                                    img_rows_bwd=None if ref_saved is None else
                                    (lambda g: refiner_bwd(model, g, ref_saved, keylen_img, B, R, seed_step, p_refine)),
                                    tok_rows=tok_rows)
        ar.touch('layer_norm_emb.weight', 'layer_norm_emb.bias', 'position_embeddings.weight')
        if not has_text_embed:
            ar.touch('embeddings.weight')
        d_ximg = d_text = None
        if R > 0:
            ops.gemm_wgrad(de, ximg16, ar.g('image_embeddings.image_embeddings.weight'))
            ar.touch(*[n for n in ar.names if n.startswith('image_embeddings.')])
            if want_dximg:
                d_ximg = ops.gemm_nt(de, _transposed(ar.w('image_embeddings.image_embeddings.weight')), L.EPI_NONE)
                d_ximg = d_ximg.view(R, B, 2048).float()
        if has_text_embed:
            d_text = tok_rows.view(T, B, d).transpose(0, 1).float()
            tok_rows = None
        if langs is not None:
            npad = (model.n_langs + 7) // 8 * 8
            onehot = torch.zeros((T * B, npad), dtype=BF16, device=tok_rows.device)
            onehot.scatter_(1, langs.view(-1, 1), 1.0)
            dl = torch.zeros((npad, d), dtype=torch.float32, device=tok_rows.device)
            ops.gemm_wgrad(onehot, tok_rows, dl)
            ar.g('cross_lang_embeddings.weight').add_(dl[:model.n_langs])
            ar.touch('cross_lang_embeddings.weight')
        if positions is not None:
            gpos = ar.g('position_embeddings.weight')
            rows32 = tok_rows.float()
            gpos.index_add_(0, positions.reshape(-1), rows32)
            gpos[:T].sub_(rows32.view(T, B, d).sum(dim=1))
        if (langs is not None or positions is not None) and (hook is None or not hook.active):
            ops.scatter_add_token_rows(tok_rows, x.contiguous().view(-1), ar.g('embeddings.weight'), model.pad_index)
            tok_rows = None
        if hook is not None:
            hook.embed_done(last, ids=x if tok_rows is not None else None, rows=tok_rows, n_max=ctx.tok_rows_max)
        return (None, None, None, None, d_ximg, None, None, None, None, None, None, None, d_text, None, None, None)


class ImageStreamFn(torch.autograd.Function):

    @staticmethod
    def forward(ctx, anchor, model, x_img, lengths, image_loc, langs, p_drop, seed_step, p_refine=None, track=False):
        ar = model.arena()
        ar.refresh()
        dev = ar.device
        d = model.dim
        R, B = x_img.shape[0], x_img.shape[1]
        seed = lambda kind: rng.stream_seed(model.base_seed, seed_step, _site(kind))
        ximg16 = ops.cast_bf16(x_img.to(dev).contiguous().view(R * B, 2048))
        loc = image_loc.to(dev).contiguous().float()
        img_proj = ops.gemm_nt(ximg16, ar.w('image_embeddings.image_embeddings.weight'), L.EPI_BIAS,
                               bias=ar.p('image_embeddings.image_embeddings.bias'))
        rows, img_saved = ops.embed_image_rows_fwd(
            img_proj, loc, ar.p('image_embeddings.image_location_embeddings.weight'),
            ar.p('image_embeddings.image_location_embeddings.bias'), ar.p('image_embeddings.LayerNorm.weight'),
            ar.p('image_embeddings.LayerNorm.bias'), B, R, d, seed_img=seed('img'), p_drop=p_drop)
        if langs is not None:
            langs = langs.to(dev).contiguous()
            rows = (rows.float() + ar.p('cross_lang_embeddings.weight')[langs.t()].reshape(B * R, d)).to(BF16)
        totlen = lengths.to(device=dev, dtype=torch.int32).contiguous()
        mask = (torch.arange(R, device=dev, dtype=torch.int32)[None, :] < totlen[:, None]).reshape(B * R, 1)
        h0 = ops.dropout_rows(rows, p_drop, seed('emb')) * mask.to(BF16)
        ref_saved = None
        if p_refine is not None:
            h0, ref_saved = refiner_fwd(model, h0.contiguous(), totlen, B, R, seed_step, p_refine)
        ctx.model = model
        ctx.saved = (ximg16, loc, img_saved, totlen, mask, langs, ref_saved)
        ctx.meta = (B, R, d, p_drop, seed_step, p_refine)
        ctx.x_img_meta = (x_img.dtype, x_img.device) if x_img.requires_grad else None
        ctx.hook = model.ddp_hook if track else None
        if ctx.hook is not None:
            ctx.hook.stream_forward()
        return h0

    @staticmethod
    def backward(ctx, dh0):
        model = ctx.model
        ar = model.arena()
        ximg16, loc, img_saved, totlen, mask, langs, ref_saved = ctx.saved
        ctx.saved = None
        B, R, d, p_drop, seed_step, p_refine = ctx.meta
        seed = lambda kind: rng.stream_seed(model.base_seed, seed_step, _site(kind))
        if ref_saved is not None:
            dh0 = refiner_bwd(model, dh0.to(BF16).contiguous(), ref_saved, totlen, B, R, seed_step, p_refine)
            ar.touch(*[n for n in ar.names if n.startswith('refine_embeddings.')])
        g = (dh0.to(BF16) * mask.to(BF16)).contiguous()
        d_rows = ops.dropout_rows(g, p_drop, seed('emb'))
        if langs is not None:
            npad = (model.n_langs + 7) // 8 * 8
# ... 542 lines not shown
```

m3p_amd/lib.py:

```python
import ctypes as C
import os

import torch

_HERE = os.path.dirname(os.path.abspath(__file__))
LIB_PATH = os.environ.get('M3P_HIP_LIB') or os.path.join(_HERE, 'libm3p_hip.so')

EPI_NONE, EPI_BIAS, EPI_BIAS_GELU, EPI_BIAS_DROP_RES, EPI_RES, EPI_DGELU, EPI_MUL, EPI_MULQ, EPI_BIAS_GELUQ, EPI_BIAS_LSE = range(10)
KERN_NT_SKINNY, KERN_NT_W8, KERN_NT_W8_QUEUE, KERN_NT_W4, KERN_NT_RING, KERN_NT_128 = range(1, 7)
KERN_WGRAD_W4_CHUNKS, KERN_WGRAD_W4_TILES, KERN_WGRAD_RING, KERN_WGRAD_128 = range(10, 14)


class M3PError(RuntimeError):
    pass


class Epilogue(C.Structure):
    _fields_ = [
        ('bias', C.c_void_p), ('aux', C.c_void_p), ('out2', C.c_void_p), ('colsum', C.c_void_p),
        ('ld_aux', C.c_int32), ('ld_out2', C.c_int32), ('scale_cols', C.c_int32), ('scale', C.c_float),
        ('alpha', C.c_float), ('seed', C.c_uint32), ('thresh24', C.c_uint32), ('inv_keep', C.c_float),
        ('descale_a', C.c_void_p), ('descale_b', C.c_void_p),
        ('out8', C.c_void_p), ('scale8', C.c_void_p), ('amax8', C.c_void_p), ('ld_out8', C.c_int32), ('out8_bf8', C.c_int32),
    ]


_p, _i, _f, _u32 = C.c_void_p, C.c_int, C.c_float, C.c_uint32

SIGNATURES = {
    'm3p_version': (C.c_char_p, []),
    'm3p_gemm_nt_bf16': (_i, [_p, _i, _p, _i, _p, _i, _i, _i, _i, _i, C.POINTER(Epilogue), _p]),
    'm3p_gemm_nt_fp8': (_i, [_p, _i, _i, _p, _i, _p, _i, _i, _i, _i, _i, C.POINTER(Epilogue), _p]),
    'm3p_quant_fp8': (_i, [_p, _i, _p, _i, _i, _i, _p, _p, _i, _p]),
    'm3p_quant_fp8_batch': (_i, [_p, _i, _i, _p]),
    'm3p_gemm_nt_streamk_f32': (_i, [_p, _i, _p, _i, _p, _i, _i, _i, _i, _f, _p]),
    'm3p_gemm_nn_streamk_f32': (_i, [_p, _i, _p, _i, _i, _p, _i, _i, _i, _i, _f, _p]),
    'm3p_gemm_nn_w4_f32': (_i, [_p, _i, _p, _i, _p, _i, _i, _i, _i, _f, _p, C.c_size_t, _p]),
    'm3p_gemm_wgrad_workspace_bytes': (C.c_size_t, []),
    'm3p_gemm_wgrad_bf16': (_i, [_p, _i, _p, _i, _p, _i, _i, _i, _i, _f, _p, C.c_size_t, _p]),
    'm3p_gemm_wgrad_store_bf16': (_i, [_p, _i, _p, _i, _p, _i, _i, _i, _i, _f, _p, C.c_size_t, _p]),
    'm3p_gemm_wgrad_pair_bf16': (_i, [_p, _i, _p, _i, _p, _i, _i, _i, _p, _i, _p, _i, _p, _i, _i, _i, _i, _f, _p, C.c_size_t, _p]),
    'm3p_layernorm_fwd': (_i, [_p, _p, _p, _p, _p, _p, _p, _i, _i, _f, _p]),
    'm3p_layernorm_bwd': (_i, [_p, _p, _p, _p, _p, _p, _p, _p, _p, _p, _p, _p, _i, _i, _u32, _u32, _f, _p]),
    'm3p_attn_fwd': (_i, [_p, _p, _p, _p, _p, _i, _i, _i, _i, _u32, _u32, _f, _p]),
    'm3p_attn_bwd': (_i, [_p, _p, _p, _p, _p, _p, _p, _p, _i, _i, _i, _i, _f, _u32, _u32, _f, _p]),
    'm3p_attn_query_fwd': (_i, [_p, _i, _p, C.c_longlong, _i, _p, _p, _i, _i, _i, _i, _i, _i, _i, _p]),
    'm3p_attn_rows_fwd': (_i, [_p, _i, _p, C.c_longlong, _i, _p, _p, _p, _i, _i, _i, _i, _i, _i, _i, _u32, _u32, _f, _p]),
    'm3p_attn_rows_bwd': (_i, [_p, _i, _p, C.c_longlong, _i, _p, _p, _p, _p, _i, _p, _i, _i, _i, _i, _i, _i, _i, _f, _u32, _u32, _f, _p]),
    'm3p_cast_f32_bf16': (_i, [_p, _p, C.c_longlong, _p]),
    'm3p_embed_assemble_fwd': (_i, [_p] * 19 + [_i, _i, _i, _i, _u32, _u32, _u32, _f, _p, _p]),
    'm3p_embed_image_rows_fwd': (_i, [_p] * 10 + [_i, _i, _i, _u32, _u32, _f, _p]),
    'm3p_embed_assemble_bwd': (_i, [_p] * 24 + [_i, _i, _i, _i, _i, _u32, _u32, _u32, _f, _i, _p]),
    'm3p_dropout_rows': (_i, [_p, _i, _p, _i, _p, _i, _i, _i, _u32, _u32, _u32, _u32, _f, _p]),
    'm3p_glu_fwd': (_i, [_p, _i, _p, _i, _i, _p]),
    'm3p_glu_bwd': (_i, [_p, _i, _p, _p, _i, _i, _p]),
    'm3p_gather_rows': (_i, [_p, _p, _p, _i, _i, _p]),
    'm3p_scatter_add_rows': (_i, [_p, _p, _p, _i, _i, _p]),
    'm3p_scatter_add_token_rows': (_i, [_p, _i, _p, _p, _i, _i, _i, _p]),
    'm3p_ce_fwd_bwd': (_i, [_p, _i, _i, _i, _p, _p, _p, _f, _f, _p]),
    'm3p_ce_colsum_workspace_bytes': (C.c_size_t, [_i, _i]),
    'm3p_ce_fwd_bwd_colsum': (_i, [_p, _i, _i, _i, _p, _p, _p, _f, _p, _p, C.c_size_t, _p]),
    'm3p_ce_lse_from_blocks': (_i, [_p, _i, _i, _p, _i, _p, _p, _p, _p, _p]),
    'm3p_ce_bwd_colsum': (_i, [_p, _i, _i, _i, _p, _p, _f, _p, _p, C.c_size_t, _p]),
    'm3p_colsum_bf16': (_i, [_p, _i, _i, _i, _p, _p, _p]),
    'm3p_sumsq_f32': (_i, [_p, C.c_longlong, _p, _p]),
    'm3p_sumsq_ranges_f32': (_i, [_p, _p, _p, _i, _p, _p]),
    'm3p_adam_step': (_i, [_p, _p, _p, _p, _p, C.c_longlong, _f, _f, _f, _f, _f, _f, _p, _f, _f, _i, _p]),
    'm3p_adam_step_ranges': (_i, [_p, _p, _p, _p, _p, _p, _p, _p, _p, _i, _f, _f, _f, _f, _f, _p, _f, _f, _p]),
    'm3p_itm_score_fwd': (_i, [_p, _p, _p, _p, _p, _i, _i, _p]),
    'm3p_itm_score_bwd': (_i, [_p, _p, _p, _p, _p, _i, _p, _p, _p, _i, _i, _p]),
    'm3p_gelu_bwd': (_i, [_p, _p, _p, C.c_longlong, _p]),
    'm3p_mse_fwd_bwd': (_i, [_p, _i, _p, _i, _p, _p, _i, _i, _f, _p]),
    'm3p_gelu_fwd': (_i, [_p, _p, _p, C.c_longlong, _p]),
    'm3p_gelu_fwd_gq': (_i, [_p, _p, _p, _i, _i, _p]),
    'm3p_gelu_fwd_q8': (_i, [_p, _p, _p, C.c_longlong, _p, _p, _p]),
    'm3p_transpose_batch_bf16': (_i, [_p, _i, _i, _p]),
    'm3p_transpose_bf16': (_i, [_p, _p, _i, _i, _i, _i, _p]),
    'm3p_set_persistent_grid': (_i, [_i]),
    'm3p_set_tile_queue': (_i, [_p, _i]),
    'm3p_gemm_nt_plan': (_i, [_i, _i, _i, _i]),
    'm3p_gemm_wgrad_plan': (_i, [_i, _i, _i]),
    'm3p_debug_set_variant': (None, [_i]),
    'm3p_debug_attn_variant': (None, [_i]),
    'm3p_seq_masks': (_i, [_p, _p, _i, _i, _p, _p, _p]),
    'm3p_mask_to_rows': (_i, [_p, _i, _i, C.c_longlong, C.c_longlong, C.c_longlong, _i, _p, _i, _p]),
    'm3p_cast_rows_f32_bf16': (_i, [_p, C.c_longlong, C.c_longlong, _i, _i, _i, _p, _p]),
    'm3p_scale_bf16_dev': (_i, [_p, _i, _p, _p, C.c_longlong, _p]),
    'm3p_axpy_dev_f32': (_i, [_p, _p, _p, C.c_longlong, _p]),
    'm3p_itm_loss_fwd_bwd': (_i, [_p, _p, _i, _i, _f, _f, _p, _p, _p]),
    'm3p_probe_mfma_16x16x32': (_i, [_p, _p, _p, _p, _p]),
    'm3p_probe_mfma_fp8_16x16x128': (_i, [_p, _p, _p, _i, _p]),
    'm3p_probe_tr16': (_i, [_p, _p, _p]),
    'm3p_probe_permlane16_swap': (_i, [_p, _p]),
}

_lib = None


def load():
    global _lib
    if _lib is not None:
        return _lib
    if not os.path.exists(LIB_PATH):
        raise M3PError('libm3p_hip.so not found at %s — build it first (make -C m3p_amd/csrc); '
                       'there is no fallback path' % LIB_PATH)
    lib = C.CDLL(LIB_PATH)
    for name, (res, args) in SIGNATURES.items():
        fn = getattr(lib, name)
        fn.restype = res
# ... 31 lines not shown
```

m3p_amd/model/transformer.py:

```python
import math
from collections import OrderedDict

import torch
import torch.nn as nn
import torch.nn.functional as F

from .. import functional as Fn

N_MAX_POSITIONS = 514

ALIGN = 64


def Embedding(num_embeddings, embedding_dim, padding_idx=None):
    m = nn.Embedding(num_embeddings, embedding_dim, padding_idx=padding_idx)
    nn.init.normal_(m.weight, mean=0, std=embedding_dim ** -0.5)
    if padding_idx is not None:
        nn.init.constant_(m.weight[padding_idx], 0)
    return m


def get_masks(slen, lengths, causal, k=None):
    bs = lengths.size(0)
    alen = torch.arange(slen, dtype=torch.long, device=lengths.device)
# ... 275 lines not shown
            return Fn.ArenaCrossWeights(self.arena())
        if self._cold_w16 is None:
            from ..decoder import _ColdWeights
            self._cold_w16 = _ColdWeights(self)
        return self._cold_w16.refresh()

    def fp8_state(self):
        if self._fp8_state is None or self._fp8_state.scale.device != self.arena().device:
            from ..fp8 import Fp8State
            self._fp8_state = Fp8State(self.n_layers, self.arena().device)
        return self._fp8_state

    def arena(self):
        if self._arena is None:
            if not self.embeddings.weight.is_cuda:
                raise RuntimeError('m3p_amd.TransformerModel runs on an MI355X only: call .cuda() first '
                                   '(there is no CPU / eager fallback for the hot path)')
            self._arena = Fn.Arena(self)
        return self._arena

    def state_dict(self, *args, **kw):
        if self.ddp_hook is not None:
            self.ddp_hook.params_ready(None)
            if getattr(self.ddp_hook, 'master_partial', False):
                raise RuntimeError('the fp32 master of the big matrices is sharded across the data-parallel ranks: call '
                                   'DataParallel.materialize_master() on EVERY rank before state_dict() '
                                   '(Trainer.save_* / end_epoch do)')
        return super().state_dict(*args, **kw)

    def load_state_dict(self, state_dict, strict=True, **kw):
        res = super().load_state_dict(state_dict, strict=strict, **kw)
        if self._arena is not None:
            self._arena.mark_master_changed()
        return res

    def forward(self, mode, **kwargs):
        if mode == 'jointfwd':
            return self.jointfwd(**kwargs)
        elif mode == 'predict':
            return self.predict(**kwargs)
        elif mode == 'crossfwd':
            return self.crossfwd(**kwargs)
        elif mode == 'transform':
            return kwargs['tensor']
        elif mode in ('fwd', 'ImageEmbed', 'GAN'):
            raise NotImplementedError("mode '%s' is outside the MI355X hot path (SURVEY.md §8f)" % mode)
        raise Exception('Unknown mode: %s' % mode)

    def _next_seed_step(self):
        self._fwd_counter += 1
        return self._fwd_counter

    def jointfwd(self, x, lengths, x_img, lengths_img, causal=False, positions=None, langs=None,
                 image_loc=None, refine_image=False, is_latent=False, text_embed=None):
        assert not causal and not is_latent, 'causal / is_latent are outside the MI355X hot path'
        T, B = x.size()
        assert lengths.size(0) == B
        R = x_img.size(0)
        p = self.dropout if self.training else 0.0
        pa = self.attention_dropout if self.training else 0.0
        p_ref = None
        if refine_image:
            assert self.n_refine_layers > 0, 'refine_image=True needs params.refine_layers > 0'
            p_ref = self.refine_dropout if self.training else 0.0
        out = self._tag_pass(Fn.EncoderFn.apply(self.layer_norm_emb.weight, self, x, lengths, x_img, lengths_img, image_loc, p, pa,
                                                self._next_seed_step(), p_ref, torch.is_grad_enabled(), text_embed))
        return out.view(B, R + T, self.dim).transpose(0, 1)

    def _tag_pass(self, out):
        out._m3p_sink = getattr(self, '_pending_sink', None)
        self._pending_sink = None
        return out

    @staticmethod
    def _drop_masked_source(src_enc, src_len, enc_mask):
        B, S = src_enc.size(0), src_enc.size(1)
        dev = src_enc.device
        ok = enc_mask.to(dev)[:, :S].bool() & (torch.arange(S, device=dev)[None, :] < src_len.to(dev)[:, None])
        order = torch.sort((~ok).to(torch.int8), dim=1, stable=True).indices
        n = ok.sum(dim=1)
        packed = torch.gather(src_enc, 1, order[:, :, None].expand(-1, -1, src_enc.size(2)))
        packed = packed * (torch.arange(S, device=dev)[None, :] < n[:, None])[:, :, None].to(packed.dtype)
        return packed, n

    def crossfwd(self, x, lengths, causal, stream_='text', src_enc=None, src_len=None, positions=None, langs=None,
                 cache=None, enc_mask=None, image_loc=None, **kw):
        if stream_ == 'img':
            assert not causal and src_enc is None and cache is None and positions is None
            assert image_loc is not None and kw.get('image_dist') is None, \
                'the image stream runs without the class-distribution embedding'
            R, B = x.size(0), x.size(1)
            if langs is not None:
                assert self.n_langs > 1 and langs.size() == (R, B)
            p = self.dropout if self.training else 0.0
            pa = self.attention_dropout if self.training else 0.0
            p_ref = None
            if kw.get('refine_image', False):
                assert self.n_refine_layers > 0, 'refine_image=True needs params.refine_layers > 0'
                p_ref = self.refine_dropout if self.training else 0.0
            step = self._next_seed_step()
            h0 = Fn.ImageStreamFn.apply(self.layer_norm_emb.weight, self, x, lengths, image_loc, langs, p, step, p_ref,
                                        torch.is_grad_enabled())
            out = self._tag_pass(Fn.EncoderFn.apply(self.layer_norm_emb.weight, self, None, lengths, None, None, None, p, pa, step,
                                                    None, torch.is_grad_enabled(), None, None, h0))
            return out.view(B, R, self.dim).transpose(0, 1)
        assert stream_ == 'text'
        if causal:
            if enc_mask is not None:
                src_enc, src_len = self._drop_masked_source(src_enc, src_len, enc_mask)
            if torch.is_grad_enabled() and self.training:
                assert cache is None
                T, B = x.size()
                out = Fn.DecoderFn.apply(self.layer_norm_emb.weight, self, x, lengths, src_enc, src_len, langs, self.dropout,
                                         self.attention_dropout, self._next_seed_step(), positions, kw.get('text_embed'))
                return out.view(B, T, self.dim).transpose(0, 1)
            from .. import decoder
            return decoder.decoder_forward(self, x, lengths, src_enc=src_enc, src_len=src_len, positions=positions,
                                           langs=langs, cache=cache)
        assert src_enc is None and cache is None, 'the non-causal text stream takes no source encoding or cache (the mlm_step caller)'
# ... 40 lines not shown
```

m3p_amd/ops.py:

```python
import ctypes as C
import os

import torch

from . import lib as L

BF16 = torch.bfloat16
_DEBUG_CHECKS = os.environ.get('M3P_DEBUG_CHECKS') == '1'

PROFILE = None
_EPI_NAMES = ['gemm_nt/none', 'gemm_nt/bias', 'gemm_nt/bias_gelu', 'gemm_nt/bias_drop_res', 'gemm_nt/res',
              'gemm_nt/dgelu', 'gemm_nt/mul', 'gemm_nt/mulq', 'gemm_nt/bias_geluq', 'gemm_nt/bias_lse']


PROFILE_ONLY = None


def _prof_begin(key=None):
    if PROFILE is None or (PROFILE_ONLY is not None and key != PROFILE_ONLY):
        return None
    e = torch.cuda.Event(enable_timing=True)
    e.record()
    return e


def _prof_end(e0, key):
    if e0 is not None:
        e1 = torch.cuda.Event(enable_timing=True)
        e1.record()
        PROFILE.setdefault(key, []).append((e0, e1))


def _chk_bf16(*ts):
    for t in ts:
        if t is not None:
            assert t.dtype == BF16 and t.is_cuda, (t.dtype, t.device)


def gemm_nt(a, w, epilogue=L.EPI_NONE, bias=None, aux=None, out=None, out2=None, colsum=None,
            scale_cols=0, scale=1.0, alpha=1.0, seed=0, p_drop=0.0, n=None, out8=None, scale8=None, amax8=None, out8_bf8=False):
    M, K = a.shape
    N = w.shape[0] if n is None else n
    if epilogue == L.EPI_MULQ:
        _chk_bf16(a, w, out)
        assert aux is not None and aux.dtype == torch.uint8 and aux.is_contiguous() and aux.numel() == M * N
    elif epilogue == L.EPI_BIAS_LSE:
        _chk_bf16(a, w, out)
        assert out2 is not None and out2.dtype == torch.float32 and out2.is_contiguous() and out2.numel() == (N // 64) * M * 2
        assert bias is not None and 0 < scale_cols <= N
    elif epilogue == L.EPI_BIAS_GELUQ:
        _chk_bf16(a, w, out)
        assert out2 is not None and out2.dtype == torch.uint8 and out2.is_contiguous() and out2.numel() == M * N and bias is not None
    else:
        _chk_bf16(a, w, aux, out, out2)
    assert w.shape[1] == K and a.stride(1) == 1 and w.stride(1) == 1
    if out is None:
        out = torch.empty((M, N), dtype=BF16, device=a.device)
    ep = L.Epilogue()
    ep.bias = L.ptr(bias)
    ep.aux = L.ptr(aux)
    ep.out2 = L.ptr(out2)
    ep.colsum = L.ptr(colsum)
    ep.ld_aux = aux.stride(0) if (aux is not None and epilogue != L.EPI_MULQ) else 0
    ep.ld_out2 = out2.stride(0) if (out2 is not None and epilogue not in (L.EPI_BIAS_GELUQ, L.EPI_BIAS_LSE)) else 0
    ep.scale_cols = scale_cols
    if epilogue == L.EPI_BIAS_LSE:
        ep.ld_out2, ep.scale_cols = scale_cols, 0
    ep.scale = scale
    ep.alpha = alpha
    ep.seed = seed
    ep.thresh24 = L.thresh24(p_drop)
    ep.inv_keep = 1.0 / (1.0 - p_drop) if p_drop > 0 else 1.0
    if bias is not None:
        assert bias.dtype == torch.float32
    if out8 is not None:
        assert epilogue in (L.EPI_BIAS_GELUQ, L.EPI_MULQ) and out8.dtype == torch.uint8 and out8.shape == (M, N) and out8.stride(1) == 1
        ep.out8, ep.ld_out8, ep.out8_bf8 = out8.data_ptr(), out8.stride(0), 1 if out8_bf8 else 0
        ep.scale8, ep.amax8 = L.ptr(scale8), L.ptr(amax8)
    e0 = _prof_begin((_EPI_NAMES[epilogue], M, N, K))
    rc = L.load().m3p_gemm_nt_bf16(a.data_ptr(), a.stride(0), w.data_ptr(), w.stride(0), out.data_ptr(),
                                   out.stride(0), M, N, K, epilogue, C.byref(ep), L.stream())
    L.check(rc, 'm3p_gemm_nt_bf16')
    _prof_end(e0, (_EPI_NAMES[epilogue], M, N, K))
    return out


def quant_fp8(x, scale=None, amax=None, bf8=False, out=None):
    _chk_bf16(x)
    rows, cols = x.shape
    assert x.stride(1) == 1
    if out is None:
        out = torch.empty((rows, cols), dtype=torch.uint8, device=x.device)
    rc = L.load().m3p_quant_fp8(x.data_ptr(), x.stride(0), out.data_ptr(), out.stride(0), rows, cols, L.ptr(scale), L.ptr(amax),
                                1 if bf8 else 0, L.stream())
    L.check(rc, 'm3p_quant_fp8')
    return out


def quant_fp8_batch(desc, n_desc, blocks_per_matrix=512):
    L.check(L.load().m3p_quant_fp8_batch(desc.data_ptr(), n_desc, blocks_per_matrix, L.stream()), 'm3p_quant_fp8_batch')


def gemm_nt_fp8(a8, w8, epilogue=L.EPI_NONE, a_is_bf8=False, descale_a=None, descale_b=None, bias=None, aux=None, out=None,
                colsum=None, scale_cols=0, scale=1.0, seed=0, p_drop=0.0):
    assert a8.dtype == torch.uint8 and w8.dtype == torch.uint8 and a8.is_cuda and w8.is_cuda
    M, K = a8.shape
    N = w8.shape[0]
    assert w8.shape[1] == K and a8.stride(1) == 1 and w8.stride(1) == 1
    _chk_bf16(aux, out)
    if out is None:
        out = torch.empty((M, N), dtype=BF16, device=a8.device)
    ep = L.Epilogue()
    ep.bias = L.ptr(bias)
    ep.aux = L.ptr(aux)
    ep.colsum = L.ptr(colsum)
    ep.ld_aux = aux.stride(0) if aux is not None else 0
    ep.scale_cols = scale_cols
    ep.scale = scale
    ep.alpha = 1.0
    ep.seed = seed
    ep.thresh24 = L.thresh24(p_drop)
    ep.inv_keep = 1.0 / (1.0 - p_drop) if p_drop > 0 else 1.0
    ep.descale_a = L.ptr(descale_a)
    ep.descale_b = L.ptr(descale_b)
    e0 = _prof_begin(('gemm_fp8/' + _EPI_NAMES[epilogue].split('/')[1], M, N, K))
    rc = L.load().m3p_gemm_nt_fp8(a8.data_ptr(), a8.stride(0), 1 if a_is_bf8 else 0, w8.data_ptr(), w8.stride(0), out.data_ptr(),
                                  out.stride(0), M, N, K, epilogue, C.byref(ep), L.stream())
# ... 63 lines not shown
    M = dy.shape[0]
    N = dy.shape[1] if n is None else n
    K = x.shape[1] if k is None else k
    assert x.shape[0] == M and dw.shape[0] >= N and dw.shape[1] >= K
    e0 = _prof_begin(('gemm_wgrad', M, N, K))
    ws = _wgrad_workspace(dy.device)
    if dw_is_zero:
        rc = L.load().m3p_gemm_wgrad_store_bf16(dy.data_ptr(), dy.stride(0), x.data_ptr(), x.stride(0), dw.data_ptr(),
                                                dw.stride(0), M, N, K, alpha, ws.data_ptr(), ws.numel(), L.stream())
        if rc == 0:
            _prof_end(e0, ('gemm_wgrad', M, N, K))
            return True if report_store else dw
        if rc != -2:
            L.check(rc, 'm3p_gemm_wgrad_store_bf16')
        if must_store:
            raise L.M3PError('m3p_gemm_wgrad_store_bf16 declined (M3P_ENOTIMPL) a store the caller depends on: dw is not physically zero')
    rc = L.load().m3p_gemm_wgrad_bf16(dy.data_ptr(), dy.stride(0), x.data_ptr(), x.stride(0), dw.data_ptr(),
                                      dw.stride(0), M, N, K, alpha, ws.data_ptr(), ws.numel(), L.stream())
    L.check(rc, 'm3p_gemm_wgrad_bf16')
    _prof_end(e0, ('gemm_wgrad', M, N, K))
    return False if report_store else dw


def gemm_wgrad_pair(dy_a, x_a, dw_a, dy_b, x_b, dw_b, alpha=1.0):
    _chk_bf16(dy_a, x_a, dy_b, x_b)
    assert dw_a.dtype == torch.float32 and dw_b.dtype == torch.float32 and dw_a.stride(-1) == 1 and dw_b.stride(-1) == 1
    M = dy_a.shape[0]
    assert x_a.shape[0] == M and dy_b.shape[0] == M and x_b.shape[0] == M
    Na, Ka, Nb, Kb = dy_a.shape[1], x_a.shape[1], dy_b.shape[1], x_b.shape[1]
    assert dw_a.shape[0] >= Na and dw_a.shape[1] >= Ka and dw_b.shape[0] >= Nb and dw_b.shape[1] >= Kb
    e0 = _prof_begin(('gemm_wgrad_pair', M, Na + Nb, Ka))
    ws = _wgrad_workspace(dy_a.device)
    rc = L.load().m3p_gemm_wgrad_pair_bf16(dy_a.data_ptr(), dy_a.stride(0), x_a.data_ptr(), x_a.stride(0), dw_a.data_ptr(), dw_a.stride(0),
                                           Na, Ka, dy_b.data_ptr(), dy_b.stride(0), x_b.data_ptr(), x_b.stride(0), dw_b.data_ptr(),
                                           dw_b.stride(0), Nb, Kb, M, alpha, ws.data_ptr(), ws.numel(), L.stream())
    L.check(rc, 'm3p_gemm_wgrad_pair_bf16')
    _prof_end(e0, ('gemm_wgrad_pair', M, Na + Nb, Ka))


def layernorm_fwd(x, gamma, beta, rowmask=None, eps=1e-12):
    _chk_bf16(x)
    rows, d = x.shape
    assert x.is_contiguous()
    y = torch.empty_like(x)
    mean = torch.empty(rows, dtype=torch.float32, device=x.device)
    rstd = torch.empty(rows, dtype=torch.float32, device=x.device)
    rc = L.load().m3p_layernorm_fwd(x.data_ptr(), gamma.data_ptr(), beta.data_ptr(), L.ptr(rowmask), y.data_ptr(),
                                    mean.data_ptr(), rstd.data_ptr(), rows, d, eps, L.stream())
    L.check(rc, 'm3p_layernorm_fwd')
    return y, mean, rstd


def layernorm_bwd(dy_a, dy_b, x, gamma, mean, rstd, rowmask, dgamma, dbeta, dbias_drop=None,
                  want_drop=False, seed=0, p_drop=0.0):
    _chk_bf16(dy_a, dy_b, x)
    rows, d = x.shape
    dx = torch.empty_like(x)
    dx_drop = torch.empty_like(x) if want_drop else None
    rc = L.load().m3p_layernorm_bwd(dy_a.data_ptr(), L.ptr(dy_b), x.data_ptr(), gamma.data_ptr(), mean.data_ptr(),
                                    rstd.data_ptr(), L.ptr(rowmask), dx.data_ptr(), L.ptr(dx_drop),
                                    dgamma.data_ptr(), dbeta.data_ptr(), L.ptr(dbias_drop), rows, d, seed,
                                    L.thresh24(p_drop), 1.0 / (1.0 - p_drop) if p_drop > 0 else 1.0, L.stream())
    L.check(rc, 'm3p_layernorm_bwd')
    return dx, dx_drop


def attn_fwd(qkv, keylen, B, S, H, dh, seed=0, p_drop=0.0, want_mask=False):
    _chk_bf16(qkv)
    assert qkv.is_contiguous() and qkv.shape == (B * S, 3 * H * dh) and keylen.dtype == torch.int32
    ctx = torch.empty((B * S, H * dh), dtype=BF16, device=qkv.device)
    lse = torch.empty((B, H, S), dtype=torch.float32, device=qkv.device)
    mask = None
    if want_mask and p_drop > 0:
        nt = (S + 15) // 16
        mask = torch.empty((B * H, nt, nt, 4), dtype=torch.int64, device=qkv.device)
    rc = L.load().m3p_attn_fwd(qkv.data_ptr(), keylen.data_ptr(), ctx.data_ptr(), lse.data_ptr(), L.ptr(mask), B, S, H, dh,
                               seed, L.thresh24(p_drop), 1.0 / (1.0 - p_drop) if p_drop > 0 else 1.0, L.stream())
    L.check(rc, 'm3p_attn_fwd')
    return (ctx, lse, mask) if want_mask else (ctx, lse)


def attn_bwd(qkv, keylen, ctx, dctx, lse, B, S, H, dh, dbias_qkv=None, seed=0, p_drop=0.0, keepmask=None):
    _chk_bf16(qkv, ctx, dctx)
    assert dctx.is_contiguous() and ctx.is_contiguous()
    assert p_drop == 0 or keepmask is not None, 'attention backward with dropout needs the keep words of the forward pass'
    dqkv = torch.empty_like(qkv)
    rc = L.load().m3p_attn_bwd(qkv.data_ptr(), keylen.data_ptr(), ctx.data_ptr(), dctx.data_ptr(), lse.data_ptr(),
                               L.ptr(keepmask), dqkv.data_ptr(), L.ptr(dbias_qkv), B, S, H, dh, 1.0 / (dh ** 0.5), seed,
                               L.thresh24(p_drop), 1.0 / (1.0 - p_drop) if p_drop > 0 else 1.0, L.stream())
    L.check(rc, 'm3p_attn_bwd')
    return dqkv


def attn_query_fwd(q, kv, klen, B, Tq, H, dh, Lk, causal=False, pos0=0):
    _chk_bf16(q, kv)
    assert q.stride(1) == 1 and kv.dim() == 3 and kv.stride(2) == 1 and kv.shape[0] == B and kv.shape[1] >= Lk
    ctx = torch.empty((B * Tq, H * dh), dtype=BF16, device=q.device)
    rc = L.load().m3p_attn_query_fwd(q.data_ptr(), q.stride(0), kv.data_ptr(), kv.stride(0), kv.stride(1), L.ptr(klen),
                                     ctx.data_ptr(), B, Tq, H, dh, Lk, 1 if causal else 0, pos0, L.stream())
    L.check(rc, 'm3p_attn_query_fwd')
    return ctx


def attn_rows_fwd(q, kv, klen, B, Tq, H, dh, Lk, causal=False, seed=0, p_drop=0.0):
    _chk_bf16(q, kv)
    assert q.stride(1) == 1 and kv.dim() == 3 and kv.stride(2) == 1 and kv.shape[0] == B and kv.shape[1] >= Lk
    ctx = torch.empty((B * Tq, H * dh), dtype=BF16, device=q.device)
    lse = torch.empty((B, H, Tq), dtype=torch.float32, device=q.device)
    rc = L.load().m3p_attn_rows_fwd(q.data_ptr(), q.stride(0), kv.data_ptr(), kv.stride(0), kv.stride(1), L.ptr(klen),
                                    ctx.data_ptr(), lse.data_ptr(), B, Tq, H, dh, Lk, 1 if causal else 0, 0, seed,
                                    L.thresh24(p_drop), 1.0 / (1.0 - p_drop) if p_drop > 0 else 1.0, L.stream())
    L.check(rc, 'm3p_attn_rows_fwd')
    return ctx, lse


def attn_rows_bwd(q, kv, klen, dctx, lse, B, Tq, H, dh, Lk, qscale, causal=False, seed=0, p_drop=0.0, dq_out=None):
# ... 147 lines not shown
    e, mean_i, rstd_i = img_saved
    assert d_rows.dtype == BF16 and d_rows.is_contiguous() and d_rows.shape == (B * R, d)
    de = torch.empty_like(e)
    th, ik = _drop_args(p_drop)
    dummy = d_rows.data_ptr()
    args = (dummy, dummy, mean_i.data_ptr(), rstd_i.data_ptr(), g_img.data_ptr(), e.data_ptr(), mean_i.data_ptr(),
            rstd_i.data_ptr(), g_img.data_ptr(), dummy, totlen.data_ptr(), loc.data_ptr(), d_rows.data_ptr(), de.data_ptr(),
            grads['d_g_img'].data_ptr(), grads['d_be_img'].data_ptr(), grads['d_g_img'].data_ptr(), grads['d_g_img'].data_ptr(),
            None, grads['d_g_img'].data_ptr(), grads['d_be_img'].data_ptr(), grads['d_b_img'].data_ptr(),
            grads['d_b_loc'].data_ptr(), grads['d_w_loc'].data_ptr(), B, 0, R, d, -1, seed_img, 0, th, ik)
    L.check(L.load().m3p_embed_assemble_bwd(*args, 2, L.stream()), 'm3p_embed_assemble_bwd')
    return de


def embed_assemble_bwd(dh, saved, g_emb, g_img, tok, totlen, loc, grads, B, T, R, d, pad_index,
                       seed_img=0, seed_emb=0, p_drop=0.0, img_rows_bwd=None, tok_rows=None):
    z, mean_e, rstd_e, e, mean_i, rstd_i = saved
    dz = torch.empty_like(z)
    de = torch.empty_like(e)
    th, ik = _drop_args(p_drop)
    if tok_rows is not None:
        assert tok_rows.dtype == BF16 and tok_rows.is_contiguous() and tok_rows.shape == (T * B, d)
    args = (dh.data_ptr(), z.data_ptr(), mean_e.data_ptr(), rstd_e.data_ptr(), g_emb.data_ptr(), e.data_ptr(),
            mean_i.data_ptr(), rstd_i.data_ptr(), g_img.data_ptr(), tok.data_ptr(), totlen.data_ptr(), L.ptr(loc),
            dz.data_ptr(), de.data_ptr(), grads['d_g_emb'].data_ptr(), grads['d_be_emb'].data_ptr(),
            grads['d_pos'].data_ptr(), grads['d_emb'].data_ptr(), L.ptr(tok_rows), grads['d_g_img'].data_ptr(),
            grads['d_be_img'].data_ptr(), grads['d_b_img'].data_ptr(), grads['d_b_loc'].data_ptr(),
            grads['d_w_loc'].data_ptr(), B, T, R, d, pad_index, seed_img, seed_emb, th, ik)
    if img_rows_bwd is not None:
        L.check(L.load().m3p_embed_assemble_bwd(*args, 1, L.stream()), 'm3p_embed_assemble_bwd')
        dz_img = dz.view(B, R + T, d)[:, :R, :]
        dz_img.copy_(img_rows_bwd(dz_img.contiguous().view(B * R, d)).view(B, R, d))
        L.check(L.load().m3p_embed_assemble_bwd(*args, 2, L.stream()), 'm3p_embed_assemble_bwd')
        return de
    L.check(L.load().m3p_embed_assemble_bwd(*args, 0, L.stream()), 'm3p_embed_assemble_bwd')
    return de


def scatter_add_token_rows(rows, ids, dst, pad_index):
    _chk_bf16(rows)
    assert ids.dtype == torch.int64 and dst.dtype == torch.float32 and rows.stride(1) == 1 and ids.is_contiguous()
    n, d = rows.shape
    assert ids.numel() == n and dst.shape[1] == d and dst.stride(0) == d
    L.check(L.load().m3p_scatter_add_token_rows(rows.data_ptr(), rows.stride(0), ids.data_ptr(), dst.data_ptr(), n, d, int(pad_index),
                                                L.stream()), 'm3p_scatter_add_token_rows')


def gather_rows(src_base, idx, n, d):
    out = torch.empty((n, d), dtype=BF16, device=idx.device)
    L.check(L.load().m3p_gather_rows(src_base.data_ptr(), idx.data_ptr(), out.data_ptr(), n, d, L.stream()), 'm3p_gather_rows')
    return out


def scatter_add_rows(src, idx, dst_base, n, d):
    L.check(L.load().m3p_scatter_add_rows(src.data_ptr(), idx.data_ptr(), dst_base.data_ptr(), n, d, L.stream()),
            'm3p_scatter_add_rows')


def ce_fwd_bwd(logits, V, target, loss_scale, grad_scale):
    n, ld = logits.shape[0], logits.stride(0)
    row_loss = torch.empty(n, dtype=torch.float32, device=logits.device)
    assert target.dtype == torch.int64
    rc = L.load().m3p_ce_fwd_bwd(logits.data_ptr(), ld, n, V, target.data_ptr(), row_loss.data_ptr(),
                                 None, loss_scale, grad_scale, L.stream())
    L.check(rc, 'm3p_ce_fwd_bwd')
    loss_sum = (row_loss.sum() * loss_scale).reshape(1)
    return loss_sum, row_loss


_CE_WS = {}


def ce_fwd_bwd_colsum(logits, V, target, loss_scale, grad_scale):
    n, ld = logits.shape[0], logits.stride(0)
    dev = logits.device
    row_loss = torch.empty(n, dtype=torch.float32, device=dev)
    row_lse = torch.empty(n, dtype=torch.float32, device=dev)
    cs = torch.empty(ld, dtype=torch.float32, device=dev)
    need = L.load().m3p_ce_colsum_workspace_bytes(ld, n)
    ws = _CE_WS.get(dev)
    if ws is None or ws.numel() < need:
        ws = _CE_WS[dev] = torch.empty(need, dtype=torch.uint8, device=dev)
    assert target.dtype == torch.int64
    rc = L.load().m3p_ce_fwd_bwd_colsum(logits.data_ptr(), ld, n, V, target.data_ptr(), row_loss.data_ptr(), row_lse.data_ptr(),
                                        grad_scale, cs.data_ptr(), ws.data_ptr(), ws.numel(), L.stream())
    L.check(rc, 'm3p_ce_fwd_bwd_colsum')
    return (row_loss.sum() * loss_scale).reshape(1), row_loss, cs


def ce_from_block_stats(logits, V, target, stats, loss_scale, grad_scale):
    n, ld = logits.shape[0], logits.stride(0)
    dev = logits.device
    row_loss = torch.empty(n, dtype=torch.float32, device=dev)
    row_lse = torch.empty(n, dtype=torch.float32, device=dev)
    cs = torch.empty(ld, dtype=torch.float32, device=dev)
    scratch = torch.empty((32, n, 2), dtype=torch.float32, device=dev)
    assert target.dtype == torch.int64 and stats.dtype == torch.float32 and stats.shape[1] == n
    L.check(L.load().m3p_ce_lse_from_blocks(stats.data_ptr(), stats.shape[0], n, logits.data_ptr(), ld, target.data_ptr(),
                                            row_loss.data_ptr(), row_lse.data_ptr(), scratch.data_ptr(), L.stream()),
            'm3p_ce_lse_from_blocks')
    need = L.load().m3p_ce_colsum_workspace_bytes(ld, n)
    ws = _CE_WS.get(dev)
    if ws is None or ws.numel() < need:
        ws = _CE_WS[dev] = torch.empty(need, dtype=torch.uint8, device=dev)
    L.check(L.load().m3p_ce_bwd_colsum(logits.data_ptr(), ld, n, V, target.data_ptr(), row_lse.data_ptr(), grad_scale, cs.data_ptr(),
                                       ws.data_ptr(), ws.numel(), L.stream()), 'm3p_ce_bwd_colsum')
# ... 177 lines not shown
```

m3p_amd/trainer.py:

```python
import math
import os
import time
from collections import OrderedDict
from logging import getLogger

import numpy as np
import torch
import torch.nn.functional as F

from . import masking
from .collate import (batch_sentences, batch_sentences_v2, caption_collate, mt_caption_collate, ntg_collate,
                      retrieval_collate, retrieval_pretrain_collate, slide_collate)
from .distributed import DataParallel
from .optim import get_optimizer
from .utils import concat_batches, parse_lambda_config, to_cuda, update_lambdas

logger = getLogger()

_REGION_HEADS = {
    'mlm': ('embeddings.weight', 'pred_layer.proj.bias'),
    'mrm': ('transformer_obj.dense.weight', 'transformer_obj.dense.bias', 'transformer_obj.LayerNorm.weight',
            'transformer_obj.LayerNorm.bias', 'pred_obj_layer.proj.weight', 'pred_obj_layer.proj.bias'),
    'mrfr': ('mrfr_dense.weight', 'mrfr_dense.bias'),
}
# ... 539 lines not shown
        self.epoch += 1


class XTrainer(Trainer):
    def __init__(self, model, data, params):
        self.MODEL_NAMES = ['model']
        self.model = model
        self.data = data
        self.params = params
        super().__init__(data, params)

    def get_iterator(self, iter_name, lang1, lang2):
        from torch.utils.data import DataLoader, RandomSampler
        from torch.utils.data.distributed import DistributedSampler
        params = self.params
        logger.info('Creating new training data iterator (%s) ...' % ','.join(
            str(v) for v in (iter_name, lang1, lang2) if v is not None))
        dataset = self.data['cross_modal'][(lang1, lang2)]['train']
        if lang1 in ('google', 'sbu') and hasattr(dataset, 'update'):
            dataset.update(self.epoch)
        if lang1 == 'flicker' and hasattr(dataset, 'update_captions'):
            dataset.update_captions()
        sampler = RandomSampler(dataset) if getattr(params, 'n_gpu_per_node', 1) == 1 else DistributedSampler(dataset)
        if getattr(params, 'is_generation', False):
            collate = mt_caption_collate if getattr(params, 'is_mt', False) else caption_collate
        elif getattr(params, 'is_pretrain', False):
            collate = retrieval_pretrain_collate
        else:
            collate = slide_collate if getattr(params, 'is_slide', False) else retrieval_collate
        loader = DataLoader(dataset, batch_size=params.batch_size, sampler=sampler, collate_fn=collate,
                            num_workers=getattr(params, 'num_workers', 0))
        for batch in loader:
            yield batch

    def get_batch(self, iter_name, lang1, lang2=None):
        assert lang2 == 'img'
        key = (iter_name, lang1, lang2)
        iterator = self.iterators.get(key)
        if iterator is None:
            iterator = self.iterators[key] = self.get_iterator(iter_name, lang1, lang2)
        try:
            return next(iterator)
        except StopIteration:
            if getattr(self.params, 'is_pretrain', False):
                self.iterators = {}
            iterator = self.iterators[key] = self.get_iterator(iter_name, lang1, lang2)
            return next(iterator)

    def get_mask_(self, x, _labels):
        pred_mask = (_labels != -1)
        y = _labels[_labels > 0]
        return y, pred_mask

    def _itm_loss(self, relation_scores, pos_labels):
        params = self.params
        dev = relation_scores.device
        pos = to_cuda(torch.as_tensor(np.asarray(pos_labels), dtype=torch.long).reshape(-1))[0] if dev.type == 'cuda' else \
            torch.as_tensor(np.asarray(pos_labels), dtype=torch.long).reshape(-1)
        if dev.type == 'cuda':
            from . import functional as Fn
            return Fn.ItmLossFn.apply(relation_scores, pos.contiguous(), params.sample_n,
                                      float(params.multi_cls_loss_weight), float(params.bin_cls_loss_weight))
        onehot = F.one_hot(pos, params.sample_n).float().view(-1)
        scores = relation_scores.float()
        loss = 0
        if params.multi_cls_loss_weight != 0:
            loss = loss + params.multi_cls_loss_weight * F.cross_entropy(scores.view(-1, params.sample_n), pos)
        if params.bin_cls_loss_weight != 0:
            loss = loss + params.bin_cls_loss_weight * F.binary_cross_entropy_with_logits(scores.view(-1), onehot)
        return loss

    def pretrain_rel_step(self, dataset='coco', input_stream='img'):
        p = self.params
        t2i_batch, i2t_batch = self.get_batch('rel', dataset, input_stream)
        if p.t2i_flag:
            self.pretrain_under_step(t2i_batch, dataset, 't2i', 'en', p.lambda_t2i, p.lambda_mlm, p.lambda_mrm, p.lambda_mrfr)
        if p.i2t_flag:
            self.pretrain_under_step(i2t_batch, dataset, 'i2t', 'en', p.lambda_i2t, p.lambda_mlm, p.lambda_mrm, p.lambda_mrfr)

    def rel_step(self, dataset='coco', input_stream='img', lambda_1=1, lambda_2=1):
        t2i_batch, i2t_batch = self.get_batch('rel', dataset, input_stream)
        freelb = getattr(self.params, 'is_freelb', False)
        if self.params.t2i_flag:
            if freelb:
                self.freelb_t2i_step(t2i_batch, dataset, lambda_1)
            self.t2i_step(t2i_batch, dataset, lambda_1)
        if self.params.i2t_flag:
            if freelb:
                self.freelb_i2t_step(t2i_batch, dataset, lambda_1)
            self.i2t_step(i2t_batch, dataset, lambda_2)

    @staticmethod
    def _uniform_like(t):
        return torch.zeros(t.shape, dtype=torch.float32).uniform_(-1, 1).to(t.device)

    def deal_freelb_delta(self, model, input_ids, input_lengths, adv_init_mag=1e-4, norm_type='l2'):
        embeds_init = _unwrap(model).embeddings(input_ids)
        if adv_init_mag > 0:
            if norm_type == 'l2':
                dims = input_lengths * embeds_init.size(-1)
                mag = adv_init_mag / torch.sqrt(dims.float())
                delta = (self._uniform_like(embeds_init) * mag.view(-1, 1, 1)).detach()
            else:
                assert norm_type == 'linf'
                delta = self._uniform_like(embeds_init) * adv_init_mag
        else:
# ... 117 lines not shown
        if free_text:
            embeds_init, delta = self.deal_freelb_delta(model, x2.transpose(0, 1), len2)
        if free_img:
            image_delta = self.deal_image_freelb_delta(x1)
        adv_steps, tb_loss = 3, 0.0
        for astep in range(adv_steps):
            text_imb, img_imb = None, x1
            if free_text:
                delta.requires_grad_()
                text_imb = delta + embeds_init
                _unwrap(model).arena().touch('embeddings.weight')
            if free_img:
                image_delta.requires_grad_()
                img_imb = x1 + image_delta
            loss, _dec = self.get_ic_output(params, model, x2, len2, img_imb, len1, img_loc, langs, langs_img, pred_mask, y, text_imb)
            loss = loss / (1.0 * adv_steps)
            self.free_optimize(loss)
            tb_loss = tb_loss + loss.detach()
            if astep == adv_steps - 1:
                break
            if free_text:
                embeds_init, delta = self.update_freelb_delta(model, delta, embeds_init, x2.transpose(0, 1))
            if free_img:
                image_delta = self.update_image_freelb_delta(x1, image_delta)
        self._stat('FRLB-IC-%s-%s' % (dataset, input_stream), tb_loss)
        self.n_sentences += params.batch_size
        self.stats['processed_s'] += len2.size(0)
        self.stats['processed_w'] += n_words
        return tb_loss

    def freelb_t2i_step(self, batches, dataset='coco', lambda_coeff=1):
        return self._freelb_rel_step(batches, dataset, 't2i', lambda_coeff)

    def freelb_i2t_step(self, batches, dataset='coco', lambda_coeff=1):
        return self._freelb_rel_step(batches, dataset, 'i2t', lambda_coeff)

    def pretrain_under_step(self, _batch, dataset='coco', task_name='t2i', lang2='en', lambda_coeff_rel=1,
                            lambda_coeff_mlm=1, lambda_coeff_mrm=1, lambda_coeff_mrfr=1):
        params = self.params
        model = self.model
        model.train()
        if task_name == 't2i':
            (x1, len1, x1_labels), (img, img_mask, img_loc, obj_labels, pos_labels, ori_att_feats, img_ids) = _batch
        else:
            (x1, len1, x1_labels), (x2, len2), (clcm_labels, img, img_mask, img_loc, obj_labels, pos_labels,
                                                ori_att_feats, img_ids) = _batch
        img_len = img_mask.sum(dim=1)
        x_img = img.transpose(0, 1)
        img_loc = img_loc.transpose(0, 1)
        y_text, pred_mask_text = self.get_mask_(x1, x1_labels)
        mlm_on, mrm_on, mrfr_on = (len(getattr(params, k)) > 0 for k in ('cross_mlm_steps', 'cross_mrm_steps', 'cross_mrfr_steps'))
        self._dp_plan(mlm_on, expect=[h for h, on in (('mlm', mlm_on), ('mrm', mrm_on), ('mrfr', mrfr_on)) if on])
        has_mlm = mlm_on and int(y_text.numel()) > 0
        x1, len1, x_img, img_loc, img_len, y_text, pred_mask_text = to_cuda(
            x1, len1, x_img, img_loc, img_len, y_text, pred_mask_text)

        encoder_outputs = model('jointfwd', x=x1, lengths=len1, x_img=x_img, lengths_img=img_len, causal=False,
                                langs=None, image_loc=img_loc, refine_image=params.refine_image)
        total_loss = None
        R = x_img.shape[0]
        _text_out = encoder_outputs[R:]
        if has_mlm:
            _, loss = model('predict', tensor=_text_out, pred_mask=pred_mask_text, y=y_text, get_scores=False)
            self._stat('CMLM-%s' % dataset, loss)
            total_loss = _add_loss(total_loss, lambda_coeff_mlm, loss)
        _img_out = encoder_outputs[:R].transpose(0, 1)
        has_masked_region = bool((obj_labels != -1).any()) if torch.is_tensor(obj_labels) else False
        if mrm_on and has_masked_region:
            _, loss = model('predict', tensor=_img_out, pred_mask=None, y=obj_labels.reshape(-1), get_scores=False, is_obj=True)
            self._stat('MRM-%s' % dataset, loss)
            total_loss = _add_loss(total_loss, lambda_coeff_mrm, loss)
        if mrfr_on and has_masked_region:
            from . import functional as Fn
            loss = Fn.mrfr_head(_unwrap(model), _img_out, obj_labels, ori_att_feats)
            self._stat('MRFR-%s' % dataset, loss)
            total_loss = _add_loss(total_loss, lambda_coeff_mrfr, loss)
        relation_scores = model('predict', tensor=encoder_outputs.transpose(0, 1), is_relation=True)
        loss = self._itm_loss(relation_scores, pos_labels)
        self._stat('%s-%s' % (task_name, dataset), loss)
        total_loss = _add_loss(total_loss, lambda_coeff_rel, loss)

        if task_name == 'i2t' and len(params.cross_clcm_steps) > 0:
            x2c, len2c = to_cuda(x2, len2)
            encoder_outputs2 = model('jointfwd', x=x2c, lengths=len2c, x_img=x_img, lengths_img=img_len, causal=False,
                                     langs=None, image_loc=img_loc, refine_image=params.refine_image)
            relation_scores2 = model('predict', tensor=encoder_outputs2.transpose(0, 1), is_clcm=True)
            target2 = torch.as_tensor(clcm_labels).reshape(-1).to(device=relation_scores2.device, dtype=torch.float32)
            loss = F.binary_cross_entropy_with_logits(relation_scores2.view(-1).float(), target2)
            self._stat('CLCM-%s' % dataset, loss)
            total_loss = _add_loss(total_loss, 1, loss)

        self.optimize(total_loss)
        self.n_sentences += params.batch_size
        self.stats['processed_s'] += len1.size(0)
        self._pending_w.append(len1.sum())
        return total_loss

    def _rel_step(self, batches, dataset, task_name, lambda_coeff):
        assert lambda_coeff >= 0
        if lambda_coeff == 0:
            return None
        params = self.params
        model = self.model
        model.train()
        text, visual = batches[0], batches[1]
        x1, len1 = text[0], text[1]
        if len(visual) == 6:
            img, img_mask, img_loc, _obj_labels, pos_labels, _img_ids = visual
        else:
            img, img_mask, img_loc, pos_labels = visual
        self._dp_plan(False)
        img_len = img_mask.sum(dim=1)
        x_img, img_loc = img.transpose(0, 1), img_loc.transpose(0, 1)
        x1, len1, x_img, img_loc, img_len = to_cuda(x1, len1, x_img, img_loc, img_len)
        enc = model('jointfwd', x=x1, lengths=len1, x_img=x_img, lengths_img=img_len, causal=False, langs=None,
                    image_loc=img_loc, refine_image=params.refine_image)
        enc = enc.transpose(0, 1)
        relation_scores = model('predict', tensor=enc, is_relation=True)
        loss = self._itm_loss(relation_scores, pos_labels)
        self._stat('%s-%s' % (task_name, dataset), loss)
        self.optimize(lambda_coeff * loss)
        bs = len1.size(0)
        self.n_sentences += params.batch_size
        self.stats['processed_s'] += bs
        self.stats['processed_w'] += bs * enc.size(1)
        return loss

    def t2i_step(self, batches, dataset='coco', lambda_coeff=1):
        return self._rel_step(batches, dataset, 't2i', lambda_coeff)

    def i2t_step(self, batches, dataset='coco', lambda_coeff=1):
        return self._rel_step(batches, dataset, 'i2t', lambda_coeff)

    def slide_step(self, dataset='slide', input_stream='img', lambda_coeff=1):
        assert lambda_coeff >= 0
        if lambda_coeff == 0:
            return None
        params = self.params
# ... 19 lines not shown
```

Before: 7964 sequences/s.

## Compute last encoder layer only for rows consumed by output heads

Adds an OutputRows descriptor built from the MLM prediction mask, region labels and the first token, so the encoder can compact the final layer's row-wise work to the rows the heads actually read. The rows are padded to a 256-row tile. A place_rows kernel scatters the results back into the full output and fills unused rows with NaN. GEMM and layernorm-backward dropout take an rng_rows remap so dropout masks stay identical to the uncompacted path. Building the masks adds host-side work per step, and the index tensors are copied to the device each step.

```diff
diff --git a/include/m3p_hip.h b/include/m3p_hip.h
--- a/include/m3p_hip.h
+++ b/include/m3p_hip.h
@@ -51,6 +51,7 @@
   float* amax8;
   int32_t ld_out8;
   int32_t out8_bf8;
+  const int32_t* rng_rows;
 } M3PEpilogue;
 
 M3P_API int m3p_gemm_nt_bf16(const void* A, int lda, const void* W, int ldw, void* C, int ldc,
@@ -89,6 +90,11 @@
                               const float* mean, const float* rstd, const uint8_t* rowmask,
                               void* dx, void* dx_drop, float* dgamma, float* dbeta, float* dbias_drop,
                               int rows, int d, uint32_t seed, uint32_t thresh24, float inv_keep, void* stream);
+M3P_API int m3p_layernorm_bwd_rows(const void* dy_a, const void* dy_b, const void* x, const float* gamma,
+                                   const float* mean, const float* rstd, const uint8_t* rowmask,
+                                   void* dx, void* dx_drop, float* dgamma, float* dbeta, float* dbias_drop,
+                                   int rows, int d, uint32_t seed, uint32_t thresh24, float inv_keep,
+                                   const int32_t* rng_rows, void* stream);
 
 
 M3P_API int m3p_attn_fwd(const void* qkv, const int32_t* keylen, void* ctx, float* lse, uint64_t* keepmask,
@@ -141,6 +147,8 @@
 
 
 M3P_API int m3p_gather_rows(const void* src, const int32_t* idx, void* dst, int n, int d, void* stream);
+M3P_API int m3p_place_rows(const void* src, const int32_t* inv, void* dst, int rows, int d, int n, uint32_t fill_bits,
+                           void* stream);
 M3P_API int m3p_scatter_add_rows(const void* src, const int32_t* idx, void* dst, int n, int d, void* stream);
 M3P_API int m3p_scatter_add_token_rows(const void* rows, int ld_rows, const int64_t* ids, float* dst, int n, int d,
                                        int pad_index, void* stream);
diff --git a/m3p_amd/csrc/gemm.hip b/m3p_amd/csrc/gemm.hip
--- a/m3p_amd/csrc/gemm.hip
+++ b/m3p_amd/csrc/gemm.hip
@@ -46,7 +46,8 @@
   }
   if (EPI == M3P_EPI_BIAS_DROP_RES) {
     if (ep.thresh24) {
-      const uint32_t base = (uint32_t)m * (uint32_t)N + (uint32_t)n;
+      const uint32_t mr = ep.rng_rows ? (uint32_t)ep.rng_rows[m] : (uint32_t)m;
+      const uint32_t base = mr * (uint32_t)N + (uint32_t)n;
       bool kp[4];
       m3p_keep_run<4>(base, ep.seed, ep.thresh24, kp);
 #pragma unroll
@@ -303,13 +304,19 @@
   load_aux_rows_finish<EPI, SW>(lane, r1, t, auxv);
 }
 
-template <int EPI, bool SW = false, bool ALDS = false>
+constexpr int M3P_EPI_DROP_RES_ROWS = 10;
+template <int EPI, bool SW = false, bool ALDS = false, bool NOROWS = false>
 __device__ __forceinline__ void epilogue_half_write(const M3PEpilogue& ep, int N, int mrow0, int nw, char* r1, const f32x4 (&rows)[2][4],
                                                     const f32x4 (&biasv)[4], const bf16x4 (&auxv)[2][4], int lane, f32x4 (&csum)[4],
                                                     bf16x4 (&ukeep)[2][4], const float* gtab = nullptr) {
   const int fr = lane & 15, fg = lane >> 4;
   constexpr bool kAux = (EPI == M3P_EPI_BIAS_DROP_RES || EPI == M3P_EPI_RES || EPI == M3P_EPI_DGELU || EPI == M3P_EPI_MUL);
   const float alpha = (ep.alpha == 0.f) ? 1.f : ep.alpha;
+  uint32_t drow[2] = {(uint32_t)(mrow0 + fr), (uint32_t)(mrow0 + 16 + fr)};
+  if (EPI == M3P_EPI_BIAS_DROP_RES && !NOROWS && ep.rng_rows != nullptr) {
+    drow[0] = (uint32_t)ep.rng_rows[mrow0 + fr];
+    drow[1] = (uint32_t)ep.rng_rows[mrow0 + 16 + fr];
+  }
 #pragma unroll
   for (int j = 0; j < 4; ++j) {
     const int n = nw + j * 16 + fg * 4;
@@ -334,7 +341,7 @@
         for (int r = 0; r < 4; ++r) v[r] = gelu_erf_f((float)ukeep[ii][j][r]);
       }
       if (EPI == M3P_EPI_BIAS_DROP_RES && ep.thresh24) {
-        const uint32_t base = (uint32_t)mrow * (uint32_t)N + (uint32_t)n;
+        const uint32_t base = drow[ii] * (uint32_t)N + (uint32_t)n;
         bool kp[4];
         m3p_keep_even<4>(base, ep.seed, ep.thresh24, kp);
 #pragma unroll
@@ -1805,11 +1812,13 @@
 #undef M3P_LGKM0
 }
 
-template <int EPI>
+template <int EPIX>
 __global__ __launch_bounds__(256)
 void gemm_nt_w4_kernel(const bf16* __restrict__ A, int lda, const bf16* __restrict__ W, int ldw,
                        bf16* __restrict__ C, int ldc, int M, int N, int K, M3PEpilogue ep,
                        int tiles_m, int tiles_n, int m_fast) {
+  constexpr bool kRows = (EPIX == M3P_EPI_DROP_RES_ROWS);
+  constexpr int EPI = kRows ? (int)M3P_EPI_BIAS_DROP_RES : EPIX;
   constexpr int BM = 256, BN = 256, KT = 64;
   constexpr int A_BYTES = BM * KT * 2, STAGE = (BM + BN) * KT * 2;
   extern __shared__ __attribute__((aligned(16))) char smem[];
@@ -2120,7 +2129,7 @@
           load_aux_rows_finish<EPI, true, true>(lane, rc, tq, aux_cur);
           if (p + 1 < 8) load_aux_rows_issue<EPI>(ep, mw + 32 * ((p + 1) & 3), nw + 64 * ((p + 1) >> 2), lane, tq);
           bf16x4 ukeep[2][4];
-          epilogue_half_write<EPI, true, true>(ep, N, mw + 32 * rg, nw + 64 * ch, rc, rows, ch ? bias_hi : bias_lo, aux_cur, lane, csum, ukeep);
+          epilogue_half_write<EPI, true, true, !kRows>(ep, N, mw + 32 * rg, nw + 64 * ch, rc, rows, ch ? bias_hi : bias_lo, aux_cur, lane, csum, ukeep);
           u32x4 R[4];
           epilogue_rows_read<true>(rc, lane, R);
           lgkm_wait_rows<true>(R, false);
@@ -2368,8 +2377,10 @@
     constexpr int BM = 256, BN = 256;
     const int tiles_m = (M + BM - 1) / BM, tiles_n = (N + BN - 1) / BN;
     const size_t lds = 2 * (BM + BN) * 128 + 4 * EP_HALF;
-    auto kern = gemm_nt_w4_kernel<EPI>;
-    static bool attr_set = false;
+    const bool rows = (EPI == M3P_EPI_BIAS_DROP_RES && ep.rng_rows != nullptr);
+    auto kern = rows ? gemm_nt_w4_kernel<(EPI == M3P_EPI_BIAS_DROP_RES ? M3P_EPI_DROP_RES_ROWS : EPI)> : gemm_nt_w4_kernel<EPI>;
+    static bool attr_set_both[2] = {false, false};
+    bool& attr_set = attr_set_both[rows ? 1 : 0];
     if (!attr_set) {
       hipError_t e = hipFuncSetAttribute((const void*)kern, hipFuncAttributeMaxDynamicSharedMemorySize, (int)lds);
       if (e != hipSuccess) return (int)e;
diff --git a/m3p_amd/csrc/heads.hip b/m3p_amd/csrc/heads.hip
--- a/m3p_amd/csrc/heads.hip
+++ b/m3p_amd/csrc/heads.hip
@@ -11,6 +11,20 @@
     const int r = (int)(i / nchunk), c = (int)(i - (size_t)r * nchunk);
     *reinterpret_cast<bf16x4*>(dst + (size_t)r * d + 4 * c) =
         *reinterpret_cast<const bf16x4*>(src + (size_t)idx[r] * d + 4 * c);
+  }
+}
+__global__ __launch_bounds__(256) void place_rows_kernel(const bf16* __restrict__ src, const int32_t* __restrict__ inv,
+                                                         bf16* __restrict__ dst, int rows, int d, int n, uint32_t fill2) {
+  typedef unsigned int u32x4 __attribute__((ext_vector_type(4)));
+  const int nchunk = d >> 3;
+  const size_t total = (size_t)rows * nchunk;
+  const u32x4 fv = u32x4{fill2, fill2, fill2, fill2};
+  for (size_t i = (size_t)blockIdx.x * blockDim.x + threadIdx.x; i < total; i += (size_t)gridDim.x * blockDim.x) {
+    const int r = (int)(i / nchunk), c = (int)(i - (size_t)r * nchunk);
+    const int j = inv[r];
+    u32x4 v = fv;
+    if (j >= 0 && j < n) v = *reinterpret_cast<const u32x4*>(src + (size_t)j * d + 8 * c);
+    *reinterpret_cast<u32x4*>(dst + (size_t)r * d + 8 * c) = v;
   }
 }
 __global__ __launch_bounds__(256) void scatter_add_rows_kernel(const bf16* __restrict__ src, const int32_t* __restrict__ idx,
@@ -336,6 +350,19 @@
   return M3P_OK;
 }
 
+int m3p_place_rows(const void* src, const int32_t* inv, void* dst, int rows, int d, int n, uint32_t fill_bits, void* stream) {
+  if (rows <= 0) return M3P_OK;
+  if (d <= 0 || (d % 8) != 0 || n < 0 || !inv || !dst || (n > 0 && !src) || ((uintptr_t)src & 15) || ((uintptr_t)dst & 15))
+    return M3P_EINVAL;
+  const size_t total = (size_t)rows * (d / 8);
+  const int blocks = (int)((total + 255) / 256 < 8192 ? (total + 255) / 256 : 8192);
+  const uint32_t f = fill_bits & 0xFFFFu;
+  hipLaunchKernelGGL(place_rows_kernel, dim3(blocks), dim3(256), 0, (hipStream_t)stream, (const bf16*)src, inv, (bf16*)dst, rows, d, n,
+                     f | (f << 16));
+  M3P_CHECK_LAUNCH();
+  return M3P_OK;
+}
+
 int m3p_scatter_add_rows(const void* src, const int32_t* idx, void* dst, int n, int d, void* stream) {
   if (n <= 0) return M3P_OK;
   if ((d % 4) != 0) return M3P_EINVAL;
diff --git a/m3p_amd/csrc/layernorm.hip b/m3p_amd/csrc/layernorm.hip
--- a/m3p_amd/csrc/layernorm.hip
+++ b/m3p_amd/csrc/layernorm.hip
@@ -65,7 +65,8 @@
                    const float* __restrict__ gamma, const float* __restrict__ mean, const float* __restrict__ rstd,
                    const uint8_t* __restrict__ rowmask, bf16* __restrict__ dx, bf16* __restrict__ dx_drop,
                    float* __restrict__ dgamma, float* __restrict__ dbeta, float* __restrict__ dbias_drop,
-                   int rows, int d, uint32_t seed, uint32_t thresh24, float inv_keep) {
+                   int rows, int d, uint32_t seed, uint32_t thresh24, float inv_keep,
+                   const int32_t* __restrict__ rng_rows) {
   __shared__ float red[4][NI * 256];
   const int lane = threadIdx.x & 63, wib = threadIdx.x >> 6;
   const int wave = (blockIdx.x * blockDim.x + threadIdx.x) >> 6;
@@ -114,7 +115,7 @@
         if (dx_drop || dbias_drop) {
           bf16x4 ob = bf16x4{(bf16)o[0], (bf16)o[1], (bf16)o[2], (bf16)o[3]};
           f32x4 od;
-          const uint32_t base = (uint32_t)r * (uint32_t)d + 4u * (uint32_t)c;
+          const uint32_t base = (uint32_t)(rng_rows ? rng_rows[r] : r) * (uint32_t)d + 4u * (uint32_t)c;
           bool kp[4] = {true, true, true, true};
           if (thresh24) m3p_keep_even<4>(base, seed, thresh24, kp);
 #pragma unroll
@@ -150,7 +151,8 @@
                       const float* __restrict__ gamma, const float* __restrict__ mean, const float* __restrict__ rstd,
                       const uint8_t* __restrict__ rowmask, bf16* __restrict__ dx, bf16* __restrict__ dx_drop,
                       float* __restrict__ dgamma, float* __restrict__ dbeta, float* __restrict__ dbias_drop,
-                      int rows, uint32_t seed, uint32_t thresh24, float inv_keep) {
+                      int rows, uint32_t seed, uint32_t thresh24, float inv_keep,
+                      const int32_t* __restrict__ rng_rows) {
   constexpr int D = 256 * NC;
   __shared__ float red[8][D];
   const int sub = threadIdx.x & 31, hw = threadIdx.x >> 5;
@@ -175,6 +177,7 @@
     const size_t ro = (size_t)r * D;
     const float mu = mean[r], rs = rstd[r];
     const float mk = rowmask ? (rowmask[r] ? 1.f : 0.f) : 1.f;
+    const uint32_t rr = rng_rows ? (uint32_t)rng_rows[r] : (uint32_t)r;
     float dyv[NC][8], xh[NC][8];
     float s1 = 0.f, s2 = 0.f;
 #pragma unroll
@@ -206,7 +209,7 @@
       for (int e = 0; e < 8; ++e) ob[e] = (bf16)((dyv[i][e] * g[i][e] - c1 - xh[i][e] * c2) * rs);
       *reinterpret_cast<bf16x8*>(dx + ro + c) = ob;
       if (dx_drop || dbias_drop) {
-        const uint32_t base = (uint32_t)r * (uint32_t)D + (uint32_t)c;
+        const uint32_t base = rr * (uint32_t)D + (uint32_t)c;
         bool kp[8] = {true, true, true, true, true, true, true, true};
         if (thresh24) m3p_keep_even<8>(base, seed, thresh24, kp);
 #pragma unroll
@@ -266,10 +269,10 @@
   return M3P_OK;
 }
 
-int m3p_layernorm_bwd(const void* dy_a, const void* dy_b, const void* x, const float* gamma, const float* mean,
-                      const float* rstd, const uint8_t* rowmask, void* dx, void* dx_drop, float* dgamma,
-                      float* dbeta, float* dbias_drop, int rows, int d, uint32_t seed, uint32_t thresh24,
-                      float inv_keep, void* stream) {
+int m3p_layernorm_bwd_rows(const void* dy_a, const void* dy_b, const void* x, const float* gamma, const float* mean,
+                           const float* rstd, const uint8_t* rowmask, void* dx, void* dx_drop, float* dgamma,
+                           float* dbeta, float* dbias_drop, int rows, int d, uint32_t seed, uint32_t thresh24,
+                           float inv_keep, const int32_t* rng_rows, void* stream) {
   if (rows <= 0 || d <= 0 || (d % 4) != 0 || d > 2048) return M3P_EINVAL;
   if (!dy_a || !x || !dx || !dgamma || !dbeta) return M3P_EINVAL;
   if (((uintptr_t)x & 7) || ((uintptr_t)dy_a & 7) || ((uintptr_t)dx & 7) || ((uintptr_t)gamma & 15)) return M3P_EINVAL;
@@ -279,11 +282,11 @@
     if (d == 768)
       hipLaunchKernelGGL(ln_bwd_hw_kernel<3>, dim3(blocks_hw), dim3(256), 0, st, (const bf16*)dy_a, (const bf16*)dy_b,
                          (const bf16*)x, gamma, mean, rstd, rowmask, (bf16*)dx, (bf16*)dx_drop, dgamma, dbeta, dbias_drop,
-                         rows, seed, thresh24, inv_keep);
+                         rows, seed, thresh24, inv_keep, rng_rows);
     else
       hipLaunchKernelGGL(ln_bwd_hw_kernel<4>, dim3(blocks_hw), dim3(256), 0, st, (const bf16*)dy_a, (const bf16*)dy_b,
                          (const bf16*)x, gamma, mean, rstd, rowmask, (bf16*)dx, (bf16*)dx_drop, dgamma, dbeta, dbias_drop,
-                         rows, seed, thresh24, inv_keep);
+                         rows, seed, thresh24, inv_keep, rng_rows);
     M3P_CHECK_LAUNCH();
     return M3P_OK;
   }
@@ -291,7 +294,7 @@
 #define M3P_LN_BWD(NI)                                                                                     \
   hipLaunchKernelGGL(ln_bwd_kernel<NI>, dim3(blocks), dim3(256), 0, st, (const bf16*)dy_a,                 \
                      (const bf16*)dy_b, (const bf16*)x, gamma, mean, rstd, rowmask, (bf16*)dx,              \
-                     (bf16*)dx_drop, dgamma, dbeta, dbias_drop, rows, d, seed, thresh24, inv_keep)
+                     (bf16*)dx_drop, dgamma, dbeta, dbias_drop, rows, d, seed, thresh24, inv_keep, rng_rows)
   switch (ln_ni(d)) {
     case 1: M3P_LN_BWD(1); break;
     case 2: M3P_LN_BWD(2); break;
@@ -304,4 +307,12 @@
   return M3P_OK;
 }
 
-}
+int m3p_layernorm_bwd(const void* dy_a, const void* dy_b, const void* x, const float* gamma, const float* mean,
+                      const float* rstd, const uint8_t* rowmask, void* dx, void* dx_drop, float* dgamma,
+                      float* dbeta, float* dbias_drop, int rows, int d, uint32_t seed, uint32_t thresh24,
+                      float inv_keep, void* stream) {
+  return m3p_layernorm_bwd_rows(dy_a, dy_b, x, gamma, mean, rstd, rowmask, dx, dx_drop, dgamma, dbeta, dbias_drop, rows, d,
+                                seed, thresh24, inv_keep, nullptr, stream);
+}
+
+}
diff --git a/m3p_amd/functional.py b/m3p_amd/functional.py
--- a/m3p_amd/functional.py
+++ b/m3p_amd/functional.py
@@ -420,14 +420,64 @@
     return sink, base, rows
 
 
-N_ENC_ARGS = 16
+N_ENC_ARGS = 17
+
+ROW_TILE = 256
+COMPACT_MIN_ROWS = 4096
+
+
+def compact_rows_eligible(n_rows, M):
+    if n_rows <= 0:
+        return 0
+    n = _round_up(n_rows, ROW_TILE)
+    return n if (n >= COMPACT_MIN_ROWS and 2 * n <= M) else 0
+
+
+class OutputRows:
+
+    def __init__(self, flags):
+        flags = torch.as_tensor(flags).reshape(-1).cpu()
+        if flags.dtype != torch.bool:
+            flags = flags != 0
+        self.flags = flags
+        self.M = int(flags.numel())
+        sel = torch.nonzero(flags).view(-1)
+        self.n_rows = int(sel.numel())
+        self.n = compact_rows_eligible(self.n_rows, self.M)
+        self.idx = self.idx64 = self.inv = None
+        if self.n:
+            pad = torch.nonzero(~flags).view(-1)[:self.n - self.n_rows]
+            idx = torch.cat([sel, pad]).to(torch.int32)
+            inv = torch.full((self.M,), -1, dtype=torch.int32)
+            inv[sel] = torch.arange(self.n_rows, dtype=torch.int32)
+            self._host = (idx, inv)
+
+    @classmethod
+    def from_masks(cls, B, S, R, first=True, pred_mask=None, region_labels=None):
+        flags = torch.zeros((B, S), dtype=torch.bool)
+        if first:
+            flags[:, 0] = True
+        if pred_mask is not None:
+            flags[:, R:] |= torch.as_tensor(pred_mask).cpu().reshape(S - R, B).t() != 0
+        if region_labels is not None and R > 0:
+            flags[:, :R] |= torch.as_tensor(region_labels).cpu().reshape(B, R) != -1
+        return cls(flags)
+
+    def to(self, device):
+        if self.n and self.idx is None:
+            from .utils import to_cuda
+            with torch.cuda.device(device):
+                self.idx, self.inv = to_cuda(*self._host)
+            self.idx64 = self.idx.long()
+        assert self.idx is None or self.idx.device == torch.device(device), 'an OutputRows serves one pass on one device'
+        return self
 
 
 class EncoderFn(torch.autograd.Function):
 
     @staticmethod
     def forward(ctx, anchor, model, x, lengths, x_img, lengths_img, image_loc, p_drop, p_attn, seed_step, p_refine=None,
-                track=False, text_embed=None, langs=None, h0=None, positions=None):
+                track=False, text_embed=None, langs=None, h0=None, positions=None, out_rows=None):
         ar = model.arena()
         ready = model.ddp_hook.params_ready if model.ddp_hook is not None else (lambda key: None)
         ar.refresh(wait_params=False)
@@ -520,6 +570,12 @@
             w8, _, dws = st8.weights[(i, wsite)]
             return ops.gemm_nt_fp8(x8, w8, epi, descale_a=dxs, descale_b=dws, **kw)
 
+        rows_c = None
+        if out_rows is not None and out_rows.n and track and st8 is None and nL > 0 and d % 8 == 0 \
+                and ops.gq_eligible(M, 4 * d) == ops.gq_eligible(out_rows.n, 4 * d):
+            assert out_rows.M == M, 'out_rows was built for %d rows, this pass has %d' % (out_rows.M, M)
+            rows_c = out_rows.to(dev)
+
         for i in range(nL):
             a, f = 'attentions.%d.' % i, 'ffns.%d.' % i
             ready(('layer', i))
@@ -527,14 +583,21 @@
             ctxt, lse, kmask = ops.attn_fwd(qkv, totlen, B, S, H, dh, seed=seed('attn_p', i), p_drop=p_attn,
                                             want_mask=True)
             lse = (lse, kmask)
-            pre1 = lin(ctxt, i, 'ctx', 'wout', ar.w(a + 'out_lin.weight'), L.EPI_BIAS_DROP_RES, bias=ar.p(a + 'out_lin.bias'),
-                       aux=h, seed=seed('attn_out', i), p_drop=p_drop)
+            compact = rows_c is not None and i == nL - 1
+            Mi, ctx_in, res_in, mask_i, rr, ctx_c = M, ctxt, h, rowmask, {}, None
+            if compact:
+                Mi, rr = rows_c.n, dict(rng_rows=rows_c.idx)
+                ctx_in = ctx_c = ops.gather_rows(ctxt, rows_c.idx, Mi, d)
+                res_in = ops.gather_rows(h, rows_c.idx, Mi, d)
+                mask_i = rowmask[rows_c.idx64]
+            pre1 = lin(ctx_in, i, 'ctx', 'wout', ar.w(a + 'out_lin.weight'), L.EPI_BIAS_DROP_RES, bias=ar.p(a + 'out_lin.bias'),
+                       aux=res_in, seed=seed('attn_out', i), p_drop=p_drop, **rr)
             x1, mean1, rstd1 = ops.layernorm_fwd(pre1, ar.p('layer_norm1.%d.weight' % i), ar.p('layer_norm1.%d.bias' % i))
             hact8 = None
             u_holds_grad = False
             if (st8 is None or 'w1' not in fp8mod.FWD_SITES) and not _GELU_GRAD_IN_FWD and _GELU_BYTE_GRAD == 2 and track \
-                    and ops.gq_eligible(M, 4 * d):
-                u = torch.empty((M * 4 * d,), dtype=torch.uint8, device=dev)
+                    and ops.gq_eligible(Mi, 4 * d):
+                u = torch.empty((Mi * 4 * d,), dtype=torch.uint8, device=dev)
                 o8 = {}
                 if st8 is not None and 'w2' in fp8mod.FWD_SITES:
                     kh = st8.index(i, 'hact')
@@ -547,31 +610,34 @@
                 elif st8 is not None and 'w2' in fp8mod.FWD_SITES:
                     st8._first_use(hact, kh)
                 u_holds_grad = 'q'
-            elif M >= 1024 or st8 is not None:
+            elif Mi >= 1024 or st8 is not None:
                 u = lin(x1, i, 'x1', 'w1', ar.w(f + 'lin1.weight'), L.EPI_BIAS, bias=ar.p(f + 'lin1.bias'))
                 if st8 is not None and 'w2' in fp8mod.FWD_SITES and 'w2' not in fp8mod.BWD_SITES and not _GELU_GRAD_IN_FWD:
                     hact, hact8 = st8.gelu_quant(u, i)
-                elif st8 is None and not _GELU_GRAD_IN_FWD and _GELU_BYTE_GRAD and track and ops.gq_eligible(M, 4 * d):
+                elif st8 is None and not _GELU_GRAD_IN_FWD and _GELU_BYTE_GRAD and track and ops.gq_eligible(Mi, 4 * d):
                     hact, u = ops.gelu_fwd_gq(u)
                     u_holds_grad = 'q'
                 else:
                     u_holds_grad = _GELU_GRAD_IN_FWD or (st8 is not None and 'w2' in fp8mod.BWD_SITES)
                     hact = ops.gelu_fwd(u, grad_inplace=u_holds_grad)
             else:
-                u = torch.empty((M, 4 * d), dtype=BF16, device=dev)
+                u = torch.empty((Mi, 4 * d), dtype=BF16, device=dev)
                 hact = ops.gemm_nt(x1, ar.w(f + 'lin1.weight'), L.EPI_BIAS_GELU, bias=ar.p(f + 'lin1.bias'), out2=u)
             pre2 = lin(hact, i, 'hact', 'w2', ar.w(f + 'lin2.weight'), L.EPI_BIAS_DROP_RES, bias=ar.p(f + 'lin2.bias'),
-                       aux=x1, seed=seed('ffn', i), p_drop=p_drop, pre8=hact8)
+                       aux=x1, seed=seed('ffn', i), p_drop=p_drop, pre8=hact8, **rr)
             h_next, mean2, rstd2 = ops.layernorm_fwd(pre2, ar.p('layer_norm2.%d.weight' % i),
-                                                     ar.p('layer_norm2.%d.bias' % i), rowmask)
+                                                     ar.p('layer_norm2.%d.bias' % i), mask_i)
             if track:
-                saved_layers.append((h, qkv, ctxt, lse, pre1, mean1, rstd1, x1, u, hact, pre2, mean2, rstd2))
+                saved_layers.append((h, qkv, ctxt, lse, pre1, mean1, rstd1, x1, u, hact, pre2, mean2, rstd2, ctx_c, mask_i))
+            if compact:
+                h_next = ops.place_rows(h_next, rows_c.inv, M, ops.BF16_NAN_BITS)
             h = h_next
 
         ctx.model = model
         ctx.dims = (B, T, R, S, d, H, dh, nL)
         ctx.drop = (p_drop, p_attn, seed_step)
         ctx.u_holds_grad = nL > 0 and u_holds_grad
+        ctx.rows_c = rows_c
         ctx.saved = (tok if text_embed is not None else x, totlen, rowmask, ximg16, loc, emb_saved, saved_layers)
         ctx.refine = (ref_saved, keylen_img, p_refine)
         ctx.input_grads = (R > 0 and x_img.requires_grad and track, text_embed is not None)
@@ -595,6 +661,7 @@
         p_drop, p_attn, seed_step = ctx.drop
         x, totlen, rowmask, ximg16, loc, emb_saved, saved_layers = ctx.saved
         ctx.saved = None
+        rows_c = ctx.rows_c
         seed = lambda kind, i=0: rng.stream_seed(model.base_seed, seed_step, _site(kind, i))
         ref_saved, keylen_img, p_refine = ctx.refine
         ctx.refine = None
@@ -626,12 +693,17 @@
 
         for i in reversed(range(nL)):
             a, f = 'attentions.%d.' % i, 'ffns.%d.' % i
-            (h_in, qkv, ctxt, lse, pre1, mean1, rstd1, x1, u, hact, pre2, mean2, rstd2) = saved_layers[i]
+            (h_in, qkv, ctxt, lse, pre1, mean1, rstd1, x1, u, hact, pre2, mean2, rstd2, ctx_c, mask_i) = saved_layers[i]
             saved_layers[i] = None
-            dpre2, dY2 = ops.layernorm_bwd(dh_, None, pre2, ar.p('layer_norm2.%d.weight' % i), mean2, rstd2, rowmask,
+            compact = rows_c is not None and i == nL - 1
+            rr = {}
+            if compact:
+                rr = dict(rng_rows=rows_c.idx)
+                dh_ = ops.gather_rows(dh_.view(M, d), rows_c.idx, rows_c.n, d)
+            dpre2, dY2 = ops.layernorm_bwd(dh_, None, pre2, ar.p('layer_norm2.%d.weight' % i), mean2, rstd2, mask_i,
                                            ar.g('layer_norm2.%d.weight' % i), ar.g('layer_norm2.%d.bias' % i),
                                            dbias_drop=ar.g(f + 'lin2.bias'), want_drop=p_drop > 0,
-                                           seed=seed('ffn', i), p_drop=p_drop)
+                                           seed=seed('ffn', i), p_drop=p_drop, **rr)
             if dY2 is None:
                 dY2 = dpre2
             ops.gemm_wgrad(dY2, hact, ar.g(f + 'lin2.weight'))
@@ -658,13 +730,20 @@
             dpre1, dAO = ops.layernorm_bwd(dx1, None, pre1, ar.p('layer_norm1.%d.weight' % i), mean1, rstd1, None,
                                            ar.g('layer_norm1.%d.weight' % i), ar.g('layer_norm1.%d.bias' % i),
                                            dbias_drop=ar.g(a + 'out_lin.bias'), want_drop=p_drop > 0,
-                                           seed=seed('attn_out', i), p_drop=p_drop)
+                                           seed=seed('attn_out', i), p_drop=p_drop, **rr)
             if dAO is None:
                 dAO = dpre1
             dctx = dgrad(dAO, i, 'dao', 'wout', ar.wt[('out', i)], L.EPI_NONE)
+            if compact:
+                ops.gemm_wgrad(dAO, ctx_c, ar.g(a + 'out_lin.weight'))
+                dctx = ops.place_rows(dctx, rows_c.inv, M, 0)
+                dpre1 = ops.place_rows(dpre1, rows_c.inv, M, 0)
             dqkv = ops.attn_bwd(qkv, totlen, ctxt, dctx, lse[0], B, S, H, dh, dbias_qkv=ar.qkv_bias(i, grad=True),
                                 seed=seed('attn_p', i), p_drop=p_attn, keepmask=lse[1])
-            ops.gemm_wgrad_pair(dqkv, h_in, ar.qkv_wgrad(i), dAO, ctxt, ar.g(a + 'out_lin.weight'))
+            if compact:
+                ops.gemm_wgrad(dqkv, h_in, ar.qkv_wgrad(i))
+            else:
+                ops.gemm_wgrad_pair(dqkv, h_in, ar.qkv_wgrad(i), dAO, ctxt, ar.g(a + 'out_lin.weight'))
             dh_ = dgrad(dqkv, i, 'dqkv', 'wqkv', ar.wt[('qkv', i)], L.EPI_RES, aux=dpre1)
             del dqkv, dctx, dAO, dpre1, dx1
             ar.touch_layer(i)
@@ -673,7 +752,7 @@
         if ctx.h0_mode is not None:
             if hook is not None:
                 hook.embed_done(last, ids=None, rows=None, n_max=ctx.tok_rows_max)
-            return (None,) * 14 + (dh_.to(ctx.h0_mode), None)
+            return (None,) * 14 + (dh_.to(ctx.h0_mode), None, None)
         want_dximg, has_text_embed = ctx.input_grads
         langs, positions = ctx.langs, ctx.positions
         tok_rows = None
@@ -723,7 +802,7 @@
             tok_rows = None
         if hook is not None:
             hook.embed_done(last, ids=x if tok_rows is not None else None, rows=tok_rows, n_max=ctx.tok_rows_max)
-        return (None, None, None, None, d_ximg, None, None, None, None, None, None, None, d_text, None, None, None)
+        return (None, None, None, None, d_ximg, None, None, None, None, None, None, None, d_text, None, None, None, None)
 
 
 class ImageStreamFn(torch.autograd.Function):
diff --git a/m3p_amd/lib.py b/m3p_amd/lib.py
--- a/m3p_amd/lib.py
+++ b/m3p_amd/lib.py
@@ -22,6 +22,7 @@
         ('alpha', C.c_float), ('seed', C.c_uint32), ('thresh24', C.c_uint32), ('inv_keep', C.c_float),
         ('descale_a', C.c_void_p), ('descale_b', C.c_void_p),
         ('out8', C.c_void_p), ('scale8', C.c_void_p), ('amax8', C.c_void_p), ('ld_out8', C.c_int32), ('out8_bf8', C.c_int32),
+        ('rng_rows', C.c_void_p),
     ]
 
 
@@ -42,6 +43,7 @@
     'm3p_gemm_wgrad_pair_bf16': (_i, [_p, _i, _p, _i, _p, _i, _i, _i, _p, _i, _p, _i, _p, _i, _i, _i, _i, _f, _p, C.c_size_t, _p]),
     'm3p_layernorm_fwd': (_i, [_p, _p, _p, _p, _p, _p, _p, _i, _i, _f, _p]),
     'm3p_layernorm_bwd': (_i, [_p, _p, _p, _p, _p, _p, _p, _p, _p, _p, _p, _p, _i, _i, _u32, _u32, _f, _p]),
+    'm3p_layernorm_bwd_rows': (_i, [_p, _p, _p, _p, _p, _p, _p, _p, _p, _p, _p, _p, _i, _i, _u32, _u32, _f, _p, _p]),
     'm3p_attn_fwd': (_i, [_p, _p, _p, _p, _p, _i, _i, _i, _i, _u32, _u32, _f, _p]),
     'm3p_attn_bwd': (_i, [_p, _p, _p, _p, _p, _p, _p, _p, _i, _i, _i, _i, _f, _u32, _u32, _f, _p]),
     'm3p_attn_query_fwd': (_i, [_p, _i, _p, C.c_longlong, _i, _p, _p, _i, _i, _i, _i, _i, _i, _i, _p]),
@@ -55,6 +57,7 @@
     'm3p_glu_fwd': (_i, [_p, _i, _p, _i, _i, _p]),
     'm3p_glu_bwd': (_i, [_p, _i, _p, _p, _i, _i, _p]),
     'm3p_gather_rows': (_i, [_p, _p, _p, _i, _i, _p]),
+    'm3p_place_rows': (_i, [_p, _p, _p, _i, _i, _i, _u32, _p]),
     'm3p_scatter_add_rows': (_i, [_p, _p, _p, _i, _i, _p]),
     'm3p_scatter_add_token_rows': (_i, [_p, _i, _p, _p, _i, _i, _i, _p]),
     'm3p_ce_fwd_bwd': (_i, [_p, _i, _i, _i, _p, _p, _p, _f, _f, _p]),
diff --git a/m3p_amd/model/transformer.py b/m3p_amd/model/transformer.py
--- a/m3p_amd/model/transformer.py
+++ b/m3p_amd/model/transformer.py
@@ -351,7 +351,7 @@
         return self._fwd_counter
 
     def jointfwd(self, x, lengths, x_img, lengths_img, causal=False, positions=None, langs=None,
-                 image_loc=None, refine_image=False, is_latent=False, text_embed=None):
+                 image_loc=None, refine_image=False, is_latent=False, text_embed=None, out_rows=None):
         assert not causal and not is_latent, 'causal / is_latent are outside the MI355X hot path'
         T, B = x.size()
         assert lengths.size(0) == B
@@ -363,7 +363,8 @@
             assert self.n_refine_layers > 0, 'refine_image=True needs params.refine_layers > 0'
             p_ref = self.refine_dropout if self.training else 0.0
         out = self._tag_pass(Fn.EncoderFn.apply(self.layer_norm_emb.weight, self, x, lengths, x_img, lengths_img, image_loc, p, pa,
-                                                self._next_seed_step(), p_ref, torch.is_grad_enabled(), text_embed))
+                                                self._next_seed_step(), p_ref, torch.is_grad_enabled(), text_embed,
+                                                None, None, None, out_rows))
         return out.view(B, R + T, self.dim).transpose(0, 1)
 
     def _tag_pass(self, out):
diff --git a/m3p_amd/ops.py b/m3p_amd/ops.py
--- a/m3p_amd/ops.py
+++ b/m3p_amd/ops.py
@@ -38,7 +38,8 @@
 
 
 def gemm_nt(a, w, epilogue=L.EPI_NONE, bias=None, aux=None, out=None, out2=None, colsum=None,
-            scale_cols=0, scale=1.0, alpha=1.0, seed=0, p_drop=0.0, n=None, out8=None, scale8=None, amax8=None, out8_bf8=False):
+            scale_cols=0, scale=1.0, alpha=1.0, seed=0, p_drop=0.0, n=None, out8=None, scale8=None, amax8=None, out8_bf8=False,
+            rng_rows=None):
     M, K = a.shape
     N = w.shape[0] if n is None else n
     if epilogue == L.EPI_MULQ:
@@ -73,6 +74,10 @@
     ep.inv_keep = 1.0 / (1.0 - p_drop) if p_drop > 0 else 1.0
     if bias is not None:
         assert bias.dtype == torch.float32
+    if rng_rows is not None:
+        assert epilogue == L.EPI_BIAS_DROP_RES and rng_rows.dtype == torch.int32 and rng_rows.is_cuda \
+            and rng_rows.is_contiguous() and rng_rows.numel() == M
+        ep.rng_rows = rng_rows.data_ptr()
     if out8 is not None:
         assert epilogue in (L.EPI_BIAS_GELUQ, L.EPI_MULQ) and out8.dtype == torch.uint8 and out8.shape == (M, N) and out8.stride(1) == 1
         ep.out8, ep.ld_out8, ep.out8_bf8 = out8.data_ptr(), out8.stride(0), 1 if out8_bf8 else 0
@@ -242,16 +247,19 @@
 
 
 def layernorm_bwd(dy_a, dy_b, x, gamma, mean, rstd, rowmask, dgamma, dbeta, dbias_drop=None,
-                  want_drop=False, seed=0, p_drop=0.0):
+                  want_drop=False, seed=0, p_drop=0.0, rng_rows=None):
     _chk_bf16(dy_a, dy_b, x)
     rows, d = x.shape
+    if rng_rows is not None:
+        assert rng_rows.dtype == torch.int32 and rng_rows.is_cuda and rng_rows.is_contiguous() and rng_rows.numel() == rows
     dx = torch.empty_like(x)
     dx_drop = torch.empty_like(x) if want_drop else None
-    rc = L.load().m3p_layernorm_bwd(dy_a.data_ptr(), L.ptr(dy_b), x.data_ptr(), gamma.data_ptr(), mean.data_ptr(),
-                                    rstd.data_ptr(), L.ptr(rowmask), dx.data_ptr(), L.ptr(dx_drop),
-                                    dgamma.data_ptr(), dbeta.data_ptr(), L.ptr(dbias_drop), rows, d, seed,
-                                    L.thresh24(p_drop), 1.0 / (1.0 - p_drop) if p_drop > 0 else 1.0, L.stream())
-    L.check(rc, 'm3p_layernorm_bwd')
+    rc = L.load().m3p_layernorm_bwd_rows(dy_a.data_ptr(), L.ptr(dy_b), x.data_ptr(), gamma.data_ptr(), mean.data_ptr(),
+                                         rstd.data_ptr(), L.ptr(rowmask), dx.data_ptr(), L.ptr(dx_drop),
+                                         dgamma.data_ptr(), dbeta.data_ptr(), L.ptr(dbias_drop), rows, d, seed,
+                                         L.thresh24(p_drop), 1.0 / (1.0 - p_drop) if p_drop > 0 else 1.0,
+                                         L.ptr(rng_rows), L.stream())
+    L.check(rc, 'm3p_layernorm_bwd_rows')
     return dx, dx_drop
 
 
@@ -505,6 +513,19 @@
     return out
 
 
+BF16_NAN_BITS = 0x7FC0
+
+
+def place_rows(src, inv, rows, fill_bits=0):
+    _chk_bf16(src)
+    n, d = src.shape
+    assert src.is_contiguous() and inv.dtype == torch.int32 and inv.is_cuda and inv.is_contiguous() and inv.numel() == rows
+    out = torch.empty((rows, d), dtype=BF16, device=src.device)
+    L.check(L.load().m3p_place_rows(src.data_ptr(), inv.data_ptr(), out.data_ptr(), rows, d, n, int(fill_bits), L.stream()),
+            'm3p_place_rows')
+    return out
+
+
 def scatter_add_rows(src, idx, dst_base, n, d):
     L.check(L.load().m3p_scatter_add_rows(src.data_ptr(), idx.data_ptr(), dst_base.data_ptr(), n, d, L.stream()),
             'm3p_scatter_add_rows')
diff --git a/m3p_amd/trainer.py b/m3p_amd/trainer.py
--- a/m3p_amd/trainer.py
+++ b/m3p_amd/trainer.py
@@ -615,6 +615,14 @@
         y = _labels[_labels > 0]
         return y, pred_mask
 
+    @staticmethod
+    def _output_rows(B, R, T, pred_mask, region_labels):
+        for t in (pred_mask, region_labels):
+            if t is not None and not (torch.is_tensor(t) and not t.is_cuda):
+                return None
+        from . import functional as Fn
+        return Fn.OutputRows.from_masks(B, R + T, R, pred_mask=pred_mask, region_labels=region_labels)
+
     def _itm_loss(self, relation_scores, pos_labels):
         params = self.params
         dev = relation_scores.device
@@ -838,11 +846,13 @@
         mlm_on, mrm_on, mrfr_on = (len(getattr(params, k)) > 0 for k in ('cross_mlm_steps', 'cross_mrm_steps', 'cross_mrfr_steps'))
         self._dp_plan(mlm_on, expect=[h for h, on in (('mlm', mlm_on), ('mrm', mrm_on), ('mrfr', mrfr_on)) if on])
         has_mlm = mlm_on and int(y_text.numel()) > 0
+        out_rows = self._output_rows(x1.shape[1], x_img.shape[0], x1.shape[0], pred_mask_text if has_mlm else None,
+                                     obj_labels if (mrm_on or mrfr_on) else None)
         x1, len1, x_img, img_loc, img_len, y_text, pred_mask_text = to_cuda(
             x1, len1, x_img, img_loc, img_len, y_text, pred_mask_text)
 
         encoder_outputs = model('jointfwd', x=x1, lengths=len1, x_img=x_img, lengths_img=img_len, causal=False,
-                                langs=None, image_loc=img_loc, refine_image=params.refine_image)
+                                langs=None, image_loc=img_loc, refine_image=params.refine_image, out_rows=out_rows)
         total_loss = None
         R = x_img.shape[0]
         _text_out = encoder_outputs[R:]
@@ -869,7 +879,8 @@
         if task_name == 'i2t' and len(params.cross_clcm_steps) > 0:
             x2c, len2c = to_cuda(x2, len2)
             encoder_outputs2 = model('jointfwd', x=x2c, lengths=len2c, x_img=x_img, lengths_img=img_len, causal=False,
-                                     langs=None, image_loc=img_loc, refine_image=params.refine_image)
+                                     langs=None, image_loc=img_loc, refine_image=params.refine_image,
+                                     out_rows=self._output_rows(x2c.shape[1], x_img.shape[0], x2c.shape[0], None, None))
             relation_scores2 = model('predict', tensor=encoder_outputs2.transpose(0, 1), is_clcm=True)
             target2 = torch.as_tensor(clcm_labels).reshape(-1).to(device=relation_scores2.device, dtype=torch.float32)
             loss = F.binary_cross_entropy_with_logits(relation_scores2.view(-1).float(), target2)
```

Measured after the change: 8105 sequences/s (median of 6 runs). 1.02x the previous value.
